# finegrain-ai/refiners

Measured on AMD Instinct MI355X. Metric: sdxl_base_1024px_images_per_sec_50_ddim_steps, higher is better.
Workload: dtype bf16; 1 GPU; SDXL-base UNet CFG step, 1024x1024 (latent 2x4x128x128, 77 text tokens), DDIM-50 + 2 LoRA r16 (722 Linears) + IP-Adapter; images_per_gpu=1, parallelism=replica x1 (independent prompts, weights broadcast once), hip_graph=True, lora_mode=fused, full=False

## Files before the change

### include/mi355x_refiners.h

```cpp
#ifndef MI355X_REFINERS_H
#define MI355X_REFINERS_H

#include <stdint.h>

#ifdef __cplusplus
extern "C" {
#endif

#define MI355X_ABI_VERSION 7

enum { MI355X_F32 = 0, MI355X_BF16 = 1 };

enum {
    MI355X_OK = 0,
    MI355X_EDTYPE = -1,
    MI355X_ESHAPE = -2,
    MI355X_ELAUNCH = -3,
    MI355X_EARG = -4
};

int mi355x_abi_version(void);
int mi355x_device_info(char* buf, int32_t buflen);

#define MI355X_MAX_SEG 3
// ... 10 lines not shown
    int32_t ups;
    int32_t H, W;
    int32_t asym;
    int32_t kblocked;
} mi355x_gemm_seg;

typedef struct {
    int32_t dtype;
    int32_t M, N;
    int32_t nseg;
    int32_t conv;
    int32_t B, OH, OW;
    mi355x_gemm_seg seg[MI355X_MAX_SEG];
    void* out;
    int64_t ldo;
    const void* bias;
    const void* rowbias;
    int64_t ld_rowbias;
    int32_t rows_per_group;
    int32_t geglu;
    const void* res;
    int64_t ldres;
    const void* zeros;
    int32_t tile;
    int32_t ksplit;
    void* ws;
    int64_t ws_bytes;
    const void* prefetch[MI355X_MAX_PREFETCH];
    int64_t prefetch_bytes[MI355X_MAX_PREFETCH];
    int32_t prefetch_blocks;
    int32_t out_kblocked;
    int32_t stages;
    int32_t nt_begin;
    void* out_t;
    int64_t ldt;
    const void* ln_stats;
    int32_t ln_parts;
    float ln_eps;
    const void* ln_s;
    const void* ln_c;
    void* stats_out;
    int32_t out_f32;
    const void* lora_a[3];
    int32_t lora_nb[3];
    int32_t lora_groups;
    int32_t lora_r;
    const void* lora_b;
    const void* lora_ls;
    const void* lora_lc;
    void* lora_t;
    int32_t* lora_flags;
    const int32_t* lora_epoch;
    float* colstats_out;
    void* sk_ws;
    int32_t* sk_flags;
    int32_t sk_slots;
} mi355x_gemm_args;

int mi355x_gemm(const mi355x_gemm_args* args, void* stream);
int mi355x_epoch_bump(int32_t* epoch, void* stream);

typedef struct {
    const void* k;
    int64_t ldk;
    int64_t k_batch_stride;
    const void* vt;
    int64_t ldvt;
    int64_t vt_batch_stride;
    int32_t Lk;
    float out_scale;
} mi355x_kv_stream;

typedef struct {
    int32_t dtype;
    int32_t B, H, D, Lq;
    int32_t nstream;
    const void* q;
    int64_t ldq;
    int64_t q_batch_stride;
    void* out;
    int64_t ldo;
    int64_t o_batch_stride;
    float scale;
    mi355x_kv_stream kv[2];
} mi355x_attn_args;

int mi355x_attention(const mi355x_attn_args* args, void* stream);

typedef struct {
    int32_t dtype;
    int32_t B, H, Lq, Lk;
    int32_t Dqk, Dv;
    int32_t causal;
    const void* q;
    int64_t ldq;
    int64_t q_batch_stride;
    const void* k;
    int64_t ldk;
    int64_t k_batch_stride;
    const void* vt;
    int64_t ldvt;
    int64_t vt_batch_stride;
    void* out;
    int64_t ldo;
    int64_t o_batch_stride;
    float scale;
    float out_scale;
} mi355x_attn_general_args;

int mi355x_attention_general(const mi355x_attn_general_args* args, void* stream);

typedef struct {
    int32_t dtype;
    int32_t M, C;
    const void* x;
    int64_t ldx;
    const void* gamma;
    const void* beta;
    float eps;
    void* out;
    int64_t ldo;
} mi355x_layernorm_args;

int mi355x_layernorm(const mi355x_layernorm_args* args, void* stream);

typedef struct {
    int32_t dtype;
    int32_t B, HW, C, G;
    const void* x;
    int64_t ldx;
    const void* gamma;
    const void* beta;
    float eps;
    int32_t silu;
    void* out;
    int64_t ldo;
    float* ws;
    const float* colstats;
    const void* x2;
    int64_t ldx2;
    int32_t C1;
    const float* colstats2;
} mi355x_groupnorm_args;

int64_t mi355x_groupnorm_ws_floats(int32_t B, int32_t HW, int32_t C);
int mi355x_groupnorm(const mi355x_groupnorm_args* args, void* stream);

int mi355x_nchw_to_nhwc(int32_t dtype, const void* x, void* out, int32_t B, int32_t C, int32_t HW, int64_t ldo, void* stream);
int mi355x_nhwc_to_nchw(int32_t dtype, const void* x, void* out, int32_t B, int32_t C, int32_t HW, int64_t ldx, void* stream);
int mi355x_im2col3x3_nchw(int32_t dtype, const void* x, void* out, int32_t B, int32_t C, int32_t H, int32_t W, int64_t ldo, void* stream);
int mi355x_patchify_nchw(int32_t dtype, const void* x, void* out, int32_t B, int32_t C, int32_t H, int32_t W, int32_t P, int64_t ldo, void* stream);
int mi355x_gather_rows(int32_t dtype, const void* x, int64_t ldx, const int32_t* idx, void* out, int64_t ldo, int64_t n_rows, int32_t C, void* stream);
int mi355x_relpos_pack(int32_t dtype, const void* src, int64_t lds, void* out, int64_t ldo, int64_t M, int32_t H, int32_t d, int32_t S1, int32_t S2,
                       int32_t Lp, int32_t Dq, void* stream);
int mi355x_pointwise_nchw(int32_t dtype, const void* x, const void* w, const void* bias, void* out, int32_t B, int32_t Ci, int32_t Co,
                          int64_t HW, void* stream);
int mi355x_concat2(int32_t dtype, const void* a, int64_t lda, int32_t C1, const void* b, int64_t ldb, int32_t C2,
                   void* out, int64_t ldo, int64_t M, void* stream);
int mi355x_axpby(int32_t dtype, const void* a, float alpha, const void* b, float beta, void* out, int64_t n, void* stream);
int mi355x_softmax_rows(int32_t dtype, const float* s, int64_t lds, void* out, int64_t ldo, int64_t M, int32_t L, int32_t Lp, float scale,
                        void* stream);
int mi355x_colsum_rows(int32_t dtype, const void* p, int64_t ldp, int32_t M, int32_t L, float* acc, int32_t accumulate, float scale, void* stream);
int mi355x_sag_degrade(int32_t dtype, const void* x, const void* eps, const float* mass, int32_t ah, int32_t aw, const float* coef, const float* w1,
                       int32_t ksize, void* out, int32_t n, int32_t C, int32_t h, int32_t w, void* stream);
int mi355x_silu(int32_t dtype, const void* x, void* out, int64_t n, void* stream);

// ... 56 lines not shown
```

### refiners_amd/csrc/attention.hip

```cpp
#include "common.cuh"
#include "../../include/mi355x_refiners.h"
#include <type_traits>

namespace {

struct KvP {
    const char* k;
    const char* vt;
    int64_t ldkb, kbsb;
    int64_t ldvtb, vtbsb;
    int Lk;
    float out_scale;
};

struct AttnP {
    int B, H, Lq, nstream;
    const char* q;
    int64_t ldqb, qbsb;
    char* out;
    int64_t ldob, obsb;
    float c;
    float thr;
    KvP kv[2];
    int qtiles;
    int xcd;
};

MI_DEV void xswap16(float& a, float& b) { asm("s_nop 1\n\tv_permlane16_swap_b32 %0, %1" : "+v"(a), "+v"(b)); }
MI_DEV void xswap32(float& a, float& b) { asm("s_nop 1\n\tv_permlane32_swap_b32 %0, %1" : "+v"(a), "+v"(b)); }
template <bool PL> MI_DEV float group_max(float x) {
    if constexpr (PL) {
        float a = x, b = x;
        xswap16(a, b);
        a = fmaxf(a, b), b = a;
        xswap32(a, b);
        return fmaxf(a, b);
    } else {
        x = fmaxf(x, __shfl_xor(x, 16));
        return fmaxf(x, __shfl_xor(x, 32));
    }
}
template <bool PL> MI_DEV float group_sum(float x) {
    if constexpr (PL) {
        float a = x, b = x;
        xswap16(a, b);
        a = a + b, b = a;
        xswap32(a, b);
        return a + b;
    } else {
        x += __shfl_xor(x, 16);
        return x + __shfl_xor(x, 32);
    }
}

template <typename T, int NW, int NSTREAM, bool GLDS, int NJQ, int RD = 2, int OPT = 0, int ABL = 0, int KVS = 1>
__global__ __launch_bounds__(NW * 64) __attribute__((amdgpu_waves_per_eu(sizeof(T) == 2 ? 2 : 1))) void attn_kernel(const AttnP p) {
    constexpr int D = 64, BKV = 64, BQW = 16 * NJQ;
    constexpr int ES = sizeof(T);
    constexpr int ROWB = D * ES;
    constexpr int CPR = ROWB / 16;
    constexpr int NTHR = NW * 64;
    constexpr int TILEB = 64 * ROWB;
    constexpr int STAGE = 2 * TILEB;
    constexpr int NST = GLDS ? 3 : 2;
    constexpr int PD = NST - 1;
    constexpr int LI = 64 * CPR / NTHR;
    constexpr int LPS = 2 * LI;
    constexpr int NS = D / DT<T>::KSTEP;
    constexpr bool IS_BF16 = (ES == 2);
    static_assert(64 * CPR % NTHR == 0, "loader mismatch");
    static_assert(KVS == 1 || (KVS == 2 && NSTREAM == 1 && !GLDS && NW % 2 == 0), "key-split: one stream, register-staged loader");
    constexpr int QW = NW / KVS;
    constexpr int TT = 4 / KVS;
    extern __shared__ __attribute__((aligned(16))) char smem[];

    const int tid = threadIdx.x, lane = tid & 63, wid = wave_id();
    const int g = lane >> 4, c16 = lane & 15;
    int bid = p.xcd ? xcd_remap(blockIdx.x, gridDim.x) : blockIdx.x;
    const int qt = bid % p.qtiles;
    bid /= p.qtiles;
    const int h = bid % p.H;
    const int b = bid / p.H;
    const int qg = KVS == 1 ? wid : wid % QW, kg = KVS == 1 ? 0 : wid / QW;
    const int q0 = qt * (BQW * QW) + qg * BQW;

    frag_t qf[NJQ][NS];
#pragma unroll
    for (int jq = 0; jq < NJQ; ++jq) {
        int qr = q0 + 16 * jq + c16;
        qr = qr < p.Lq ? qr : p.Lq - 1;
        const char* qp = p.q + (int64_t)b * p.qbsb + (int64_t)qr * p.ldqb + (int64_t)h * ROWB;
#pragma unroll
        for (int s = 0; s < NS; ++s) {
            if constexpr (ABL & 32) qf[jq][s] = frag_t{lane, s, jq, 0x3c003c00};
            else qf[jq][s] = *reinterpret_cast<const frag_t*>(qp + (4 * s + g) * 16);
        }
    }

    int lrow[LI], lcoff[LI], vrowd[LI];
#pragma unroll
    for (int it = 0; it < LI; ++it) {
        const int q = it * NTHR + tid, row = q / CPR, pch = q % CPR;
        lrow[it] = IS_BF16 ? k_row_key(row) : row;
        lcoff[it] = (pch ^ swz<ROWB>(row)) << 4;
        const int j = row >> 4, a = (row >> 2) & 3, bb = row & 3;
        vrowd[it] = 16 * a + 4 * j + bb;
    }
    frag_t kr[RD][LI], vr[RD][LI];
// ... 304 lines not shown
            }
        }

        if constexpr (KVS == 2) {
            constexpr int NV = 18 * NJQ;
            float* mg = reinterpret_cast<float*>(smem) + (qg * NV) * 64 + lane;
            if (kg == 1) {
#pragma unroll
                for (int jq = 0; jq < NJQ; ++jq) {
#pragma unroll
                    for (int i = 0; i < 4; ++i)
#pragma unroll
                        for (int r = 0; r < 4; ++r) mg[(jq * 18 + 4 * i + r) * 64] = o[i][jq][r];
                    mg[(jq * 18 + 16) * 64] = mrun[jq];
                    mg[(jq * 18 + 17) * 64] = lsum[jq];
                }
            }
            __syncthreads();
            if (kg == 0) {
#pragma unroll
                for (int jq = 0; jq < NJQ; ++jq) {
                    const float m1 = mg[(jq * 18 + 16) * 64], l1 = mg[(jq * 18 + 17) * 64];
                    const float m = fmaxf(mrun[jq], m1);
                    const float a0 = fast_exp2((mrun[jq] - m) * p.c), a1 = fast_exp2((m1 - m) * p.c);
                    lsum[jq] = lsum[jq] * a0 + l1 * a1;
#pragma unroll
                    for (int i = 0; i < 4; ++i)
#pragma unroll
                        for (int r = 0; r < 4; ++r) o[i][jq][r] = o[i][jq][r] * a0 + mg[(jq * 18 + 4 * i + r) * 64] * a1;
                }
            }
        }

#pragma unroll
        for (int jq = 0; jq < NJQ; ++jq) {
            float l;
            if constexpr (ONES) l = lacc[jq][0];
            else l = group_sum<(OPT & 1) != 0>(lsum[jq]);
            const float inv = kv.out_scale / l;
#pragma unroll
            for (int i = 0; i < 4; ++i) {
                if constexpr (NSTREAM > 1) res[i][jq] += o[i][jq] * inv;
                else res[i][jq] = o[i][jq] * inv;
            }
        }
    }

    constexpr int EPC = DT<T>::EPC;
#pragma unroll
    for (int jq = 0; jq < NJQ; ++jq) {
        const int qr = q0 + 16 * jq + c16;
        if (qr >= p.Lq || kg != 0) continue;
        if constexpr (ABL & 16) {
            if (res[0][jq][0] != 12345.678f) continue;
        }
        T* op = reinterpret_cast<T*>(p.out + (int64_t)b * p.obsb + (int64_t)qr * p.ldob + (int64_t)h * ROWB) + 16 * g;
        float v[16];
#pragma unroll
        for (int i = 0; i < 4; ++i)
#pragma unroll
            for (int r = 0; r < 4; ++r) v[4 * i + r] = res[i][jq][r];
#pragma unroll
        for (int c = 0; c < 16 / EPC; ++c) {
            Vec16<T> ov;
#pragma unroll
            for (int e = 0; e < EPC; ++e) ov.set(e, v[c * EPC + e]);
            store16<T>(op + c * EPC, ov);
        }
    }
}

typedef __amdgpu_buffer_rsrc_t rsrc_t;
MI_DEV rsrc_t make_rsrc(const char* base, int64_t bytes) {
    const uint64_t b = reinterpret_cast<uint64_t>(base);
    const uint32_t lo = __builtin_amdgcn_readfirstlane((uint32_t)b), hi = __builtin_amdgcn_readfirstlane((uint32_t)(b >> 32));
    const int64_t nb = bytes < 0x7ffffff0 ? bytes : 0x7ffffff0;
    const int n = __builtin_amdgcn_readfirstlane((int)nb);
    return __builtin_amdgcn_make_buffer_rsrc(reinterpret_cast<void*>(((uint64_t)hi << 32) | lo), (short)0, n, 0x00020000);
}
MI_DEV void blds16(rsrc_t rs, char* lds_wave_base, uint32_t voff, uint32_t soff) {
    __builtin_amdgcn_raw_ptr_buffer_load_lds(rs, (lptr_t)lds_wave_base, 16, (int)voff, (int)soff, 0, 0);
}

template <int NJQ, int SCHED, int ABL = 0, bool DMA = false, bool FOLD = false>
__global__ __launch_bounds__(256) __attribute__((amdgpu_waves_per_eu(2))) void attn_pipe_kernel(const AttnP p) {
    using T = bf16_t;
    constexpr int NW = 4, D = 64, BKV = 64, BQW = 16 * NJQ, ES = 2, ROWB = D * ES, CPR = ROWB / 16, NTHR = NW * 64, TILEB = 64 * ROWB;
    constexpr int LI = 64 * CPR / NTHR, NS = 2;
    extern __shared__ __attribute__((aligned(16))) char smem[];

    const int tid = threadIdx.x, lane = tid & 63, wid = wave_id();
    const int g = lane >> 4, c16 = lane & 15;
    int bid = p.xcd ? xcd_remap(blockIdx.x, gridDim.x) : blockIdx.x;
    const int qt = bid % p.qtiles;
    bid /= p.qtiles;
    const int h = bid % p.H;
    const int b = bid / p.H;
    const int q0 = qt * (BQW * NW) + wid * BQW;

    frag_t qf[NJQ][NS];
#pragma unroll
    for (int jq = 0; jq < NJQ; ++jq) {
        int qr = q0 + 16 * jq + c16;
        qr = qr < p.Lq ? qr : p.Lq - 1;
        const char* qp = p.q + (int64_t)b * p.qbsb + (int64_t)qr * p.ldqb + (int64_t)h * ROWB;
#pragma unroll
        for (int s = 0; s < NS; ++s) {
            qf[jq][s] = *reinterpret_cast<const frag_t*>(qp + (4 * s + g) * 16);
            if constexpr (FOLD) {
                bf16x8 qv = __builtin_bit_cast(bf16x8, qf[jq][s]);
#pragma unroll
                for (int e = 0; e < 8; ++e) qv[e] = (bf16_t)((float)qv[e] * p.c);
                qf[jq][s] = __builtin_bit_cast(frag_t, qv);
            }
        }
    }

    const KvP& kv = p.kv[0];
    const int Lk = kv.Lk;
    const int ntile = (Lk + BKV - 1) / BKV;
    const char* kbase = kv.k + (int64_t)b * kv.kbsb + (int64_t)h * ROWB;
    const char* vbase = kv.vt + (int64_t)h * D * kv.ldvtb + (int64_t)b * kv.vtbsb;
    char* const kbuf = smem;
    char* const vbuf = smem + 2 * TILEB;
    uint32_t koff[LI], koff_last[LI], voff[LI];
#pragma unroll
    for (int it = 0; it < LI; ++it) {
        const int q = it * NTHR + tid, row = q / CPR, pch = q % CPR;
        const int key = k_row_key(row);
        const int coff = (pch ^ swz<ROWB>(row)) << 4;
        const int last = Lk - 1 - (ntile - 1) * BKV;
        koff[it] = (uint32_t)(key * (int)kv.ldkb + coff);
        koff_last[it] = (uint32_t)((key < last ? key : last) * (int)kv.ldkb + coff);
        const int j = row >> 4, a = (row >> 2) & 3, bb = row & 3;
        voff[it] = (uint32_t)((16 * a + 4 * j + bb) * (int)kv.ldvtb + coff);
    }

    const rsrc_t krs = make_rsrc(kbase, (int64_t)(Lk - 1) * kv.ldkb + ROWB);
    const rsrc_t vrs = make_rsrc(vbase, (int64_t)(D - 1) * kv.ldvtb + (int64_t)ntile * BKV * ES);
    auto dma_k = [&](int tile, int buf) {
        const uint32_t soff = (uint32_t)(tile * BKV) * (uint32_t)kv.ldkb;
        const bool lastt = tile == ntile - 1;
#pragma unroll
        for (int it = 0; it < LI; ++it) blds16(krs, kbuf + buf * TILEB + (it * NTHR + wid * 64) * 16, lastt ? koff_last[it] : koff[it], soff);
    };
    auto dma_v = [&](int tile, int buf) {
        const uint32_t soff = (uint32_t)(tile * BKV * ES);
#pragma unroll
        for (int it = 0; it < LI; ++it) blds16(vrs, vbuf + buf * TILEB + (it * NTHR + wid * 64) * 16, voff[it], soff);
    };
    frag_t kr[LI], vr[LI];
    auto load_k = [&](int tile) {
        const char* base = kbase + (int64_t)tile * BKV * kv.ldkb;
        const bool lastt = tile == ntile - 1;
#pragma unroll
        for (int it = 0; it < LI; ++it) kr[it] = *reinterpret_cast<const frag_t*>(base + (lastt ? koff_last[it] : koff[it]));
    };
    auto load_v = [&](int tile) {
        const char* base = vbase + (int64_t)tile * BKV * ES;
#pragma unroll
        for (int it = 0; it < LI; ++it) vr[it] = *reinterpret_cast<const frag_t*>(base + voff[it]);
    };
    auto commit_k = [&](int buf) {
#pragma unroll
        for (int it = 0; it < LI; ++it) *reinterpret_cast<frag_t*>(kbuf + buf * TILEB + (it * NTHR + tid) * 16) = kr[it];
    };
    auto commit_v = [&](int buf) {
#pragma unroll
        for (int it = 0; it < LI; ++it) *reinterpret_cast<frag_t*>(vbuf + buf * TILEB + (it * NTHR + tid) * 16) = vr[it];
    };

    f32x4 o[4][NJQ], lacc[NJQ];
#pragma unroll
    for (int jq = 0; jq < NJQ; ++jq) {
        lacc[jq] = f32x4{0.f, 0.f, 0.f, 0.f};
#pragma unroll
        for (int i = 0; i < 4; ++i) o[i][jq] = f32x4{0.f, 0.f, 0.f, 0.f};
    }
    float mrun[NJQ];
#pragma unroll
    for (int jq = 0; jq < NJQ; ++jq) mrun[jq] = FOLD ? 0.f : -INFINITY;
    const frag_t ones = frag_t{0x3f803f80, 0x3f803f80, 0x3f803f80, 0x3f803f80};

    auto qk = [&](const char* ks, f32x4(&sn)[4][NJQ]) {
        frag_t kf[4][NS];
#pragma unroll
        for (int t = 0; t < 4; ++t)
#pragma unroll
            for (int s = 0; s < NS; ++s) kf[t][s] = lds_read_frag(ks, tile_off<ROWB>(16 * t + c16, 4 * s + g));
#pragma unroll
        for (int t = 0; t < 4; ++t) {
#pragma unroll
// ... 602 lines not shown
            const int kv0 = (sidx ? sl - nt0 : sl) * BKV;
            if (Lk - kv0 <= 32) tile(smem + sl * STAGE, kv0, Lk, std::true_type{});
            else tile(smem + sl * STAGE, kv0, Lk, std::false_type{});
        }
    }
    finish(p.kv[NSTREAM - 1].out_scale);

#pragma unroll
    for (int jq = 0; jq < NJQ; ++jq) {
        const int qr = q0 + 16 * jq + c16;
        if (qr >= p.Lq) continue;
        T* op = reinterpret_cast<T*>(p.out + (int64_t)b * p.obsb + (int64_t)qr * p.ldob + (int64_t)h * ROWB) + 16 * g;
#pragma unroll
        for (int c = 0; c < 2; ++c) {
            Vec16<T> ov;
#pragma unroll
            for (int e = 0; e < 8; ++e) ov.set(e, res[(c * 8 + e) >> 2][jq][e & 3]);
            store16<T>(op + c * 8, ov);
        }
    }
}

int g_attn_short_q16 = 0;

int g_attn_short_dma = 1;

template <typename T, int NSTREAM, int NJQ, bool DMA>
auto short_kernel_of() {
    if constexpr (DMA) return attn_short_dma_kernel<NSTREAM, NJQ>;
    else return attn_short_kernel<T, NSTREAM, NJQ>;
}

template <typename T, int NSTREAM, int NJQ = 2, bool DMA = false>
int launch_attn_short(const AttnP& p0, int xcd, hipStream_t stream) {
    if constexpr (sizeof(T) == 2 && !DMA) {
        bool ok = g_attn_short_dma != 0;
        for (int s = 0; s < p0.nstream; ++s) ok = ok && 64 * p0.kv[s].ldkb < 0x7fffffff && 64 * p0.kv[s].ldvtb < 0x7fffffff;
        if (ok) return launch_attn_short<T, NSTREAM, NJQ, true>(p0, xcd, stream);
    }
    constexpr int LDS = 3 * 2 * 64 * 64 * sizeof(T);
    auto kfn = short_kernel_of<T, NSTREAM, NJQ, DMA>();
    static bool attr_set = false;
    if (!attr_set) {
        (void)hipFuncSetAttribute(reinterpret_cast<const void*>(kfn), hipFuncAttributeMaxDynamicSharedMemorySize, LDS);
        attr_set = true;
    }
    AttnP p = p0;
    constexpr int BQ = 64 * NJQ;
    p.qtiles = (p.Lq + BQ - 1) / BQ;
    p.xcd = xcd;
    hipLaunchKernelGGL(kfn, dim3(p.qtiles * p.H * p.B), dim3(256), LDS, stream, p);
    return hipGetLastError() == hipSuccess ? MI355X_OK : MI355X_ELAUNCH;
}

int g_attn_glds = 0;
int g_attn_depth = 1;
int g_attn_xcd = 1;
int g_attn_opt = 13;
int g_attn_abl = 0;
int g_attn_kvs = 0;

template <typename T, int NW, int NSTREAM, bool GLDS, int NJQ = 2, int RD = 2, int OPT = 0, int ABL = 0, int KVS = 1>
int launch_attn(const AttnP& p0, hipStream_t stream) {
    constexpr int LDS = (GLDS ? 3 : 2) * 2 * 64 * 64 * sizeof(T);
    auto kfn = attn_kernel<T, NW, NSTREAM, GLDS, NJQ, RD, OPT, ABL, KVS>;
    static bool attr_set = false;
    if (!attr_set) {
        (void)hipFuncSetAttribute(reinterpret_cast<const void*>(kfn), hipFuncAttributeMaxDynamicSharedMemorySize, LDS);
        attr_set = true;
    }
    AttnP p = p0;
    constexpr int BQ = 16 * NJQ * NW / KVS;
    p.qtiles = (p.Lq + BQ - 1) / BQ;
    p.xcd = g_attn_xcd;
    const int grid = p.qtiles * p.H * p.B;
    hipLaunchKernelGGL(kfn, dim3(grid), dim3(NW * 64), LDS, stream, p);
    return hipGetLastError() == hipSuccess ? MI355X_OK : MI355X_ELAUNCH;
}

int g_attn_pipe = 3;

int g_attn_pipe_fold = 0;

template <int NJQ, int SCHED, int ABL = 0, bool DMA = false, bool FOLD = false>
int launch_attn_pipe(const AttnP& p0, hipStream_t stream) {
    constexpr int LDS = 4 * 64 * 64 * 2;
    auto kfn = attn_pipe_kernel<NJQ, SCHED, ABL, DMA, FOLD>;
    static bool attr_set = false;
    if (!attr_set) {
        (void)hipFuncSetAttribute(reinterpret_cast<const void*>(kfn), hipFuncAttributeMaxDynamicSharedMemorySize, LDS);
        attr_set = true;
    }
    AttnP p = p0;
    constexpr int BQ = 16 * NJQ * 4;
    p.qtiles = (p.Lq + BQ - 1) / BQ;
    p.xcd = g_attn_xcd;
    hipLaunchKernelGGL(kfn, dim3(p.qtiles * p.H * p.B), dim3(256), LDS, stream, p);
    return hipGetLastError() == hipSuccess ? MI355X_OK : MI355X_ELAUNCH;
}

int g_attn_nw = 0;

template <typename T, int NW, int OPT>
int launch_attn_opt(const AttnP& p, hipStream_t stream) {
    if constexpr (NW != 2) {
        if (g_attn_depth == 2) {
            if constexpr (OPT != 2) {
                if (p.nstream == 2) return launch_attn<T, NW, 2, false, 2, 2, OPT>(p, stream);
            }
            if (p.nstream == 1) return launch_attn<T, NW, 1, false, 2, 2, OPT>(p, stream);
        }
    }
    if (p.nstream == 2) return launch_attn<T, NW, 2, false, 2, 1, OPT>(p, stream);
    return launch_attn<T, NW, 1, false, 2, 1, OPT>(p, stream);
}

template <typename T, int NW>
int launch_attn_nw(const AttnP& p, hipStream_t stream) {
    if constexpr (NW == 4 && sizeof(T) == 2) {
#ifdef MI355X_ATTN_PIPE_ABL
        if (g_attn_pipe && p.nstream == 1 && g_attn_abl != 0) {
            switch (g_attn_abl) {
                case 1: return launch_attn_pipe<2, 1, 1>(p, stream);
                case 2: return launch_attn_pipe<2, 1, 2>(p, stream);
                case 4: return launch_attn_pipe<2, 1, 4>(p, stream);
                case 6: return launch_attn_pipe<2, 1, 6>(p, stream);
                case 8: return launch_attn_pipe<2, 1, 8>(p, stream);
                case 16: return launch_attn_pipe<2, 1, 16>(p, stream);
                case 24: return launch_attn_pipe<2, 1, 24>(p, stream);
                case 32: return launch_attn_pipe<2, 1, 32>(p, stream);
                case 33: return launch_attn_pipe<2, 1, 33>(p, stream);
                case 39: return launch_attn_pipe<2, 1, 39>(p, stream);
                case 63: return launch_attn_pipe<2, 1, 63>(p, stream);
                case 128: return launch_attn_pipe<2, 1, 0, true>(p, stream);
                case 129: return launch_attn_pipe<2, 1, 1, true>(p, stream);
                case 134: return launch_attn_pipe<2, 1, 6, true>(p, stream);
                case 144: return launch_attn_pipe<2, 1, 16, true>(p, stream);
                case 167: return launch_attn_pipe<2, 1, 39, true>(p, stream);
                case 136: return launch_attn_pipe<2, 1, 8, true>(p, stream);
                case 152: return launch_attn_pipe<2, 1, 24, true>(p, stream);
                case 175: return launch_attn_pipe<2, 1, 47, true>(p, stream);
                case 191: return launch_attn_pipe<2, 1, 63, true>(p, stream);
                default: return MI355X_EARG;
            }
        }
#endif
    }
    if (g_attn_glds) {
        if (p.nstream == 2) return launch_attn<T, NW, 2, true>(p, stream);
        return launch_attn<T, NW, 1, true>(p, stream);
    }
    if constexpr (NW == 4 && sizeof(T) == 2) {
        if (g_attn_abl && p.nstream == 1) {
            switch (g_attn_abl) {
                case 1: return launch_attn<T, 4, 1, false, 2, 1, 0, 1>(p, stream);
                case 2: return launch_attn<T, 4, 1, false, 2, 1, 0, 2>(p, stream);
                case 4: return launch_attn<T, 4, 1, false, 2, 1, 0, 4>(p, stream);
                case 8: return launch_attn<T, 4, 1, false, 2, 1, 0, 8>(p, stream);
                case 6: return launch_attn<T, 4, 1, false, 2, 1, 0, 6>(p, stream);
                case 14: return launch_attn<T, 4, 1, false, 2, 1, 0, 14>(p, stream);
                case 15: return launch_attn<T, 4, 1, false, 2, 1, 0, 15>(p, stream);
                case 31: return launch_attn<T, 4, 1, false, 2, 1, 0, 31>(p, stream);
                case 63: return launch_attn<T, 4, 1, false, 2, 1, 0, 63>(p, stream);
                case 127: return launch_attn<T, 4, 1, false, 2, 1, 0, 127>(p, stream);
                case 16: return launch_attn<T, 4, 1, false, 2, 1, 0, 16>(p, stream);
                default: return MI355X_EARG;
            }
        }
    }
    if constexpr (NW == 4 && sizeof(T) == 2) {
        if (g_attn_pipe && p.nstream == 1 && g_attn_abl == 0 && g_attn_kvs != 2) {
            const int64_t wg128 = (int64_t)((p.Lq + 127) / 128) * p.H * p.B;
            const bool q16 = g_attn_kvs == 3 || (g_attn_kvs == 0 && wg128 <= 640 && p.kv[0].Lk >= 256);
            if (g_attn_pipe == 2) return q16 ? launch_attn_pipe<1, 0>(p, stream) : launch_attn_pipe<2, 0>(p, stream);
            if (g_attn_pipe == 3) {
                const bool dma_ok = (int64_t)p.kv[0].Lk * p.kv[0].ldkb < 0x7fffffff && 64 * p.kv[0].ldvtb < 0x7fffffff;
                if (dma_ok && g_attn_pipe_fold) return q16 ? launch_attn_pipe<1, 1, 0, true, true>(p, stream) : launch_attn_pipe<2, 1, 0, true, true>(p, stream);
                if (dma_ok) return q16 ? launch_attn_pipe<1, 1, 0, true>(p, stream) : launch_attn_pipe<2, 1, 0, true>(p, stream);
            }
            return q16 ? launch_attn_pipe<1, 1>(p, stream) : launch_attn_pipe<2, 1>(p, stream);
        }
    }
    if constexpr (NW == 4) {
        const int64_t wg128 = (int64_t)((p.Lq + 127) / 128) * p.H * p.B;
        const bool short_grid = wg128 <= 384 && p.kv[0].Lk >= 256;
        if (p.nstream == 1 && (g_attn_kvs == 3 || (g_attn_kvs == 0 && short_grid))) {
            if constexpr (sizeof(T) == 2) {
                switch (g_attn_opt) {
                    case 5: return launch_attn<T, 4, 1, false, 1, 1, 5>(p, stream);
                    case 9: return launch_attn<T, 4, 1, false, 1, 1, 9>(p, stream);
                    case 13: return launch_attn<T, 4, 1, false, 1, 1, 13>(p, stream);
                    default: break;
                }
            }
            return launch_attn<T, 4, 1, false, 1, 1, 1>(p, stream);
        }
        if (p.nstream == 1 && g_attn_kvs == 2) return (g_attn_opt & 1) ? launch_attn<T, 4, 1, false, 2, 1, 1, 0, 2>(p, stream) : launch_attn<T, 4, 1, false, 2, 1, 0, 0, 2>(p, stream);
    }
    if constexpr (NW == 4 && sizeof(T) == 2) {
        if (p.nstream == 1) {
            switch (g_attn_opt) {
                case 5: return launch_attn<T, 4, 1, false, 2, 1, 5>(p, stream);
                case 9: return launch_attn<T, 4, 1, false, 2, 1, 9>(p, stream);
                case 13: return launch_attn<T, 4, 1, false, 2, 1, 13>(p, stream);
                default: break;
            }
        }
    }
    switch (g_attn_opt & 3) {
        case 1: return launch_attn_opt<T, NW, 1>(p, stream);
        case 2: return launch_attn_opt<T, NW, 2>(p, stream);
        case 3: return launch_attn_opt<T, NW, 3>(p, stream);
        default: return launch_attn_opt<T, NW, 0>(p, stream);
    }
}

int g_attn_short = 1;

template <typename T>
int launch_attn_t(const AttnP& p, hipStream_t stream) {
    if (g_attn_short && !g_attn_glds && g_attn_nw == 0 && g_attn_abl == 0 && g_attn_kvs != 2) {
        int tiles = 0;
        for (int s = 0; s < p.nstream; ++s) tiles += (p.kv[s].Lk + 63) / 64;
        if (tiles <= 3) {
            const int64_t wg128 = (int64_t)((p.Lq + 127) / 128) * p.H * p.B;
            if (g_attn_short_q16 == 2 || (g_attn_short_q16 == 0 && wg128 <= 640))
                return p.nstream == 2 ? launch_attn_short<T, 2, 1>(p, g_attn_xcd, stream) : launch_attn_short<T, 1, 1>(p, g_attn_xcd, stream);
            return p.nstream == 2 ? launch_attn_short<T, 2>(p, g_attn_xcd, stream) : launch_attn_short<T, 1>(p, g_attn_xcd, stream);
        }
    }
    int nw = g_attn_nw;
    if (nw == 0) nw = 4;
    if (nw == 14) return p.nstream == 2 ? launch_attn<T, 4, 2, false, 1, 1>(p, stream) : launch_attn<T, 4, 1, false, 1, 1>(p, stream);
    if (nw == 18) return p.nstream == 2 ? launch_attn<T, 8, 2, false, 1, 1>(p, stream) : launch_attn<T, 8, 1, false, 1, 1>(p, stream);
    return nw == 2 ? launch_attn_nw<T, 2>(p, stream) : launch_attn_nw<T, 4>(p, stream);
}

inline bool al16(const void* p) { return (reinterpret_cast<uintptr_t>(p) & 15) == 0; }

}

extern "C" int mi355x_attention_set_nw(int v) {
    g_attn_nw = v;
    return MI355X_OK;
}

extern "C" int mi355x_attention_set_glds(int v) {
    g_attn_glds = v;
    return MI355X_OK;
}

extern "C" int mi355x_attention_set_pipeline(int tiles_in_flight, int xcd_aware) {
    const int d = tiles_in_flight & 15;
    if (d == 1 || d == 2) g_attn_depth = d;
    g_attn_opt = (tiles_in_flight >> 4) & 15;
    g_attn_abl = (tiles_in_flight >> 8) & 255;
    g_attn_kvs = (tiles_in_flight >> 16) & 3;
    g_attn_short = ((tiles_in_flight >> 18) & 1) ? 0 : 1;
    g_attn_pipe = (tiles_in_flight >> 19) & 3;
    g_attn_pipe_fold = (tiles_in_flight >> 21) & 1;
    g_attn_short_q16 = (tiles_in_flight >> 23) & 3;
    g_attn_short_dma = ((tiles_in_flight >> 25) & 1) ? 0 : 1;
    if (xcd_aware >= 0) g_attn_xcd = xcd_aware ? 1 : 0;
    return MI355X_OK;
}

extern "C" int mi355x_attention(const mi355x_attn_args* a, void* stream) {
    if (!a || !a->q || !a->out) return MI355X_EARG;
    if (a->dtype != MI355X_F32 && a->dtype != MI355X_BF16) return MI355X_EDTYPE;
    if (a->D != 64 || a->B <= 0 || a->H <= 0 || a->Lq <= 0 || a->nstream < 1 || a->nstream > 2) return MI355X_ESHAPE;
    const int es = a->dtype == MI355X_F32 ? 4 : 2;
    if (!al16(a->q) || !al16(a->out) || (a->ldq * es) % 16 || (a->ldo * es) % 16 || (a->q_batch_stride * es) % 16 ||
        (a->o_batch_stride * es) % 16)
        return MI355X_ESHAPE;
    AttnP p{};
    p.B = a->B;
    p.H = a->H;
    p.Lq = a->Lq;
    p.nstream = a->nstream;
    p.q = static_cast<const char*>(a->q);
    p.ldqb = a->ldq * es;
    p.qbsb = a->q_batch_stride * es;
    p.out = static_cast<char*>(a->out);
    p.ldob = a->ldo * es;
    p.obsb = a->o_batch_stride * es;
    p.c = a->scale * 1.44269504088896340736f;
    p.thr = p.c > 0.f ? 8.0f / p.c : 0.f;
    for (int s = 0; s < a->nstream; ++s) {
        const mi355x_kv_stream& k = a->kv[s];
        if (!k.k || !k.vt || k.Lk <= 0) return MI355X_ESHAPE;
        if (!al16(k.k) || !al16(k.vt) || (k.ldk * es) % 16 || (k.ldvt * es) % 16 || (k.k_batch_stride * es) % 16 ||
            (k.vt_batch_stride * es) % 16)
            return MI355X_ESHAPE;
        p.kv[s].k = static_cast<const char*>(k.k);
        p.kv[s].vt = static_cast<const char*>(k.vt);
        p.kv[s].ldkb = k.ldk * es;
        p.kv[s].kbsb = k.k_batch_stride * es;
        p.kv[s].ldvtb = k.ldvt * es;
        p.kv[s].vtbsb = k.vt_batch_stride * es;
        p.kv[s].Lk = k.Lk;
        p.kv[s].out_scale = k.out_scale;
    }
    hipStream_t st = static_cast<hipStream_t>(stream);
    if (a->dtype == MI355X_F32) return launch_attn_t<float>(p, st);
    return launch_attn_t<bf16_t>(p, st);
}
```

### refiners_amd/csrc/gemm.hip

```cpp
#include <climits>

#include "gemm8_kernel.cuh"
#include "gemm_kernel.cuh"

namespace mi355x {

int g_pf_blocks = 64;
int g_pf_mode = 1;
int g_tile = 0;
int g_stages = 0;
int g_lora_dbg = 0;
int g_sk_g = 0;
int g_g8_persist = 1;

namespace {
inline bool aligned16(const void* p) { return (reinterpret_cast<uintptr_t>(p) & 15) == 0; }
}

}

using namespace mi355x;

extern "C" int mi355x_set_option(const char* name, int value);
extern "C" int mi355x_set_option(const char* name, int value) {
    if (!name) return MI355X_EARG;
    if (name[0] == 'g' && name[1] == 'n') {
        extern int g_gn_wgs, g_gn_unroll;
        if (name[2] == 'w') g_gn_wgs = value;
        else g_gn_unroll = value;
        return MI355X_OK;
    }
    if (name[0] == 'g' && name[1] == '8') {
        g_g8_persist = value;
        return MI355X_OK;
    }
    if (name[0] == 's' && name[1] == 'k') {
        g_sk_g = value;
        return MI355X_OK;
    }
    if (name[0] == 's') {
        g_stages = value;
        return MI355X_OK;
    }
    if (name[0] == 'p') {
        if (name[2] == 'b') g_pf_blocks = value < 0 ? 0 : (value + 7) / 8 * 8;
        else g_pf_mode = value;
        return MI355X_OK;
    }
    if (name[0] == 'l') {
        g_lora_dbg = value;
        return MI355X_OK;
    }
    if (name[0] == 't') {
        g_tile = value;
        return MI355X_OK;
    }
    return MI355X_EARG;
}

static int g_stat_g8 = 0, g_stat_g8_lora = 0, g_stat_g9 = 0, g_stat_g11 = 0, g_stat_g12 = 0;
extern "C" int mi355x_get_stat(const char* name);
extern "C" int mi355x_get_stat(const char* name) {
    if (!name) return MI355X_EARG;
    if (name[0] == 'g' && name[1] == '8') return name[2] == 'l' ? g_stat_g8_lora : g_stat_g8;
    if (name[0] == 'g' && name[1] == '9') return g_stat_g9;
    if (name[0] == 'g' && name[1] == '1' && name[2] == '1') return g_stat_g11;
    if (name[0] == 'g' && name[1] == '1' && name[2] == '2') return g_stat_g12;
    return MI355X_EARG;
}

namespace {
__global__ void epoch_bump_kernel(int* e) {
    const int v = *e + 1;
    *e = v == 0 ? 1 : v;
}
}

extern "C" int mi355x_epoch_bump(int32_t* epoch, void* stream) {
    if (!epoch) return MI355X_EARG;
    hipLaunchKernelGGL(epoch_bump_kernel, dim3(1), dim3(1), 0, static_cast<hipStream_t>(stream), epoch);
    return hipGetLastError() == hipSuccess ? MI355X_OK : MI355X_ELAUNCH;
}

extern "C" int mi355x_gemm(const mi355x_gemm_args* a, void* stream) {
    if (!a) return MI355X_EARG;
    const bool has_t = a->out_t != nullptr;
    if (!a->out && !(has_t && a->nt_begin == 0)) return MI355X_EARG;
    if (a->dtype != MI355X_F32 && a->dtype != MI355X_BF16) return MI355X_EDTYPE;
    if (a->M <= 0 || a->N <= 0 || a->nseg < 1 || a->nseg > MI355X_MAX_SEG) return MI355X_ESHAPE;
    const int es = a->dtype == MI355X_F32 ? 4 : 2;
    const int bke = 128 / es;
    GemmP p{};
    p.M = a->M;
    p.N = a->N;
    p.nseg = a->nseg;
    p.OH = a->OH;
    p.OW = a->OW;
    if (a->conv) {
        if (!a->zeros || a->B <= 0 || a->OH <= 0 || a->OW <= 0 || (int64_t)a->B * a->OH * a->OW != a->M) return MI355X_ESHAPE;
    }
    for (int s = 0; s < a->nseg; ++s) {
        const mi355x_gemm_seg& g = a->seg[s];
        if (!g.x || !g.w || g.k <= 0 || g.k % bke) return MI355X_ESHAPE;
        const bool wkb = g.kblocked & 1, xkb = (g.kblocked & 2) != 0;
        if (xkb && a->conv) return MI355X_ESHAPE;
        if (!aligned16(g.x) || !aligned16(g.w) || (!xkb && (g.ldx * es) % 16) || (!wkb && (g.ldw * es) % 16)) return MI355X_ESHAPE;
        SegP& d = p.seg[s];
        d.wkb = wkb ? 1 : 0;
        d.xkb = xkb ? 1 : 0;
        d.x = static_cast<const char*>(g.x);
        d.w = static_cast<const char*>(g.w);
        d.ldxb = g.ldx * es;
        d.ldwb = g.ldw * es;
        {
            const int64_t taps = a->conv ? (int64_t)g.ksize * g.ksize : 1, kbytes = (int64_t)g.k * es, nkb_all = taps * (g.k / bke);
            const int64_t xrows = a->conv ? (int64_t)a->B * g.H * g.W : (int64_t)a->M;
            d.xbytes = xkb ? nkb_all * a->M * 128 : (xrows - 1) * d.ldxb + kbytes;
            d.wbytes = wkb ? nkb_all * a->N * 128 : ((int64_t)a->N - 1) * d.ldwb + taps * kbytes;
        }
        if (a->conv) {
            if ((g.ksize != 1 && g.ksize != 3) || (g.stride != 1 && g.stride != 2) || (g.ups != 1 && g.ups != 2)) return MI355X_ESHAPE;
            if (g.H <= 0 || g.W <= 0) return MI355X_ESHAPE;
            d.cpb = g.k / bke;
            d.nkb = g.ksize * g.ksize * d.cpb;
            d.ksize = g.ksize;
            d.pad = g.asym ? 0 : g.ksize / 2;
            d.stride = g.stride;
            d.ups_shift = g.ups == 2 ? 1 : 0;
            d.H = g.H;
            d.W = g.W;
        } else {
            d.cpb = 1;
            d.nkb = g.k / bke;
            d.ksize = 1;
            d.pad = 0;
            d.stride = 1;
            d.ups_shift = 0;
        }
    }
    p.out = static_cast<char*>(a->out);
    p.ldo = a->ldo;
    p.bias = static_cast<const char*>(a->bias);
    p.rowbias = static_cast<const char*>(a->rowbias);
    p.ld_rowbias = a->ld_rowbias;
    p.rows_per_group = a->rows_per_group > 0 ? a->rows_per_group : 1;
    p.geglu = a->geglu == 1 ? 1 : 0;
// ... 130 lines not shown
```

### refiners_amd/csrc/gemm_epilogue.cuh

```cuda
#pragma once
#include "gemm_params.cuh"

enum : unsigned { EPI_LN = 1, EPI_RB = 2, EPI_GELU = 4, EPI_GEGLU = 8, EPI_RES = 16, EPI_F32 = 32, EPI_ST = 64, EPI_CS = 128, EPI_ALL = 255 };
#define EPIF(bit, x) (((F) & (bit)) != 0 && (x))

namespace mi355x {

template <int BM, int NTHR_ALL>
MI_DEV void ln_rowstat(const GemmP& p, int m0, int tid_all, float* rowstat) {
    constexpr int TPR = NTHR_ALL / BM;
    static_assert(TPR >= 1 && (TPR & (TPR - 1)) == 0 && TPR <= 8, "threads per row");
    const int row = tid_all / TPR, sub = tid_all % TPR;
    const int m = min(m0 + row, p.M - 1);
    float cn = 0.f, mean = 0.f, m2 = 0.f;
    constexpr int MAXP = 24;
    const float* sp = p.ln_stats + (int64_t)m * 2;
    const int64_t pstride = (int64_t)p.M * 2;
    f32x2 st[MAXP];
#pragma unroll
    for (int i = 0; i < MAXP; ++i) {
        const int part = sub + i * TPR;
        st[i] = part < p.ln_parts ? *reinterpret_cast<const f32x2*>(sp + part * pstride) : f32x2{0.f, 0.f};
    }
#pragma unroll
// ... 325 lines not shown
    const T* bias = reinterpret_cast<const T*>(p.bias);
    const T* rowbias = reinterpret_cast<const T*>(p.rowbias);
    const T* res = reinterpret_cast<const T*>(p.res);
    float s1[4] = {0.f, 0.f, 0.f, 0.f}, s2[4] = {0.f, 0.f, 0.f, 0.f};
    const bool full4 = n + 4 <= p.N;
    if (n < p.N) {
        f32x4 part[2][MAXS];
#pragma unroll
        for (int r = 0; r < 2; ++r) {
            const int m = min(bm * 32 + ty * 2 + r, p.M - 1);
#pragma unroll
            for (int s = 0; s < MAXS; ++s) {
                part[r][s] = f32x4{0.f, 0.f, 0.f, 0.f};
                if (s < p.ksplit) {
                    const float* pp = p.partial + ((int64_t)s * p.M + m) * p.N + n;
                    if (full4) part[r][s] = *reinterpret_cast<const f32x4*>(pp);
                    else
                        for (int q = 0; q < 4; ++q)
                            if (n + q < p.N) part[r][s][q] = pp[q];
                }
            }
        }
#pragma unroll
        for (int r = 0; r < 2; ++r) {
            const int m = bm * 32 + ty * 2 + r;
            if (m >= p.M) break;
            float v[4] = {0.f, 0.f, 0.f, 0.f};
#pragma unroll
            for (int s = 0; s < MAXS; ++s)
                if (s < p.ksplit) v[0] += part[r][s][0], v[1] += part[r][s][1], v[2] += part[r][s][2], v[3] += part[r][s][3];
            for (int s = MAXS; s < p.ksplit; ++s) {
                const float* pp = p.partial + ((int64_t)s * p.M + m) * p.N + n;
                for (int q = 0; q < 4; ++q)
                    if (n + q < p.N) v[q] += pp[q];
            }
#pragma unroll
            for (int q = 0; q < 4; ++q) {
                const int nn = n + q;
                if (nn >= p.N) break;
                float val = v[q];
                if (bias) val += to_f32(bias[nn]);
                if (rowbias) val += to_f32(rowbias[(int64_t)(m / p.rows_per_group) * p.ld_rowbias + nn]);
                if (p.gelu) val = epi_act(p.gelu, val);
                if (res) val += to_f32(res[(int64_t)m * p.ldres + nn]);
                const T o = from_f32<T>(val);
                out[(int64_t)m * p.ldo + nn] = o;
                const float f = to_f32(o);
                s1[q] += f;
                s2[q] += f * f;
            }
        }
    }
    if (p.colstats) {
        if (ty > 0) {
#pragma unroll
            for (int q = 0; q < 4; ++q) {
                red[ty - 1][tx][q] = s1[q];
                red[ty - 1][tx][4 + q] = s2[q];
            }
        }
        __syncthreads();
        if (ty == 0 && n < p.N) {
#pragma unroll
            for (int q = 0; q < 4; ++q) {
                if (n + q >= p.N) break;
                float a = s1[q], b = s2[q];
#pragma unroll
                for (int j = 0; j < 15; ++j) {
                    a += red[j][tx][q];
                    b += red[j][tx][4 + q];
                }
                f32x2 st = {a, b};
                *reinterpret_cast<f32x2*>(p.colstats + ((int64_t)bm * p.N + n + q) * 2) = st;
            }
        }
    }
}

extern int g_pf_blocks;
extern int g_pf_mode;
extern int g_tile;
extern int g_stages;
extern int g_lora_dbg;


inline void plan_grid(GemmP& q, int BM, int BN, bool conv, int kg) {
    const GemmP& p = q;
    q.tiles_n = (p.N + BN - 1) / BN;
    q.tiles_m = (p.M + BM - 1) / BM;
    double kx = 0, kw = 0;
    for (int sgi = 0; sgi < p.nseg; ++sgi) {
        const SegP& sg = p.seg[sgi];
        kw += sg.nkb;
        kx += conv ? (double)sg.nkb / (sg.ksize * sg.ksize) : (double)sg.nkb;
    }
    const double bx_ = (double)p.M * kx, bw_ = (double)p.N * kw;
    double best = bx_ + 8.0 * bw_;
    q.pn = 0;
    q.hm = q.hn = 0;
    if (8.0 * bx_ + bw_ < best) {
        best = 8.0 * bx_ + bw_;
        q.pn = -1;
    }
    for (int pm = 2; pm <= 4; pm *= 2) {
        const int pn = 8 / pm;
        if (q.tiles_m % pm || q.tiles_n % pn) continue;
        const double cost = pn * bx_ + pm * bw_;
        if (cost < best) {
            best = cost;
            q.pn = pn;
            q.hm = q.tiles_m / pm;
            q.hn = q.tiles_n / pn;
        }
    }
    q.grid0 = q.tiles_m * q.tiles_n;
    bool any_pf = false;
    for (int i = 0; i < MI355X_MAX_PREFETCH; ++i) any_pf = any_pf || (q.pf_ptr[i] && q.pf_bytes[i] > 0);
    if (!any_pf || g_pf_blocks == 0) q.pf_blocks = 0;
    else if (q.pf_blocks <= 0) q.pf_blocks = g_pf_blocks;
    q.pf_blocks = (q.pf_blocks + 7) / 8 * 8;
    if (kg > 1) q.pf_blocks = (q.pf_blocks / 2 + 7) / 8 * 8;
    q.pf_mode = g_pf_mode;
}

}
```

### refiners_amd/csrc/gemm_kernel.cuh

```cuda
#pragma once
#include "gemm_epilogue.cuh"
#include "gemm_lora_producer.cuh"

namespace mi355x {

#ifndef MI355X_GEMM_PRIO
#define MI355X_GEMM_PRIO 1
#endif
#ifndef MI355X_LORA_TT
#define MI355X_LORA_TT 1
#endif
#ifndef MI355X_LORA_TT_HOOKS
#define MI355X_LORA_TT_HOOKS 0
#endif
#ifndef MI355X_LORA64_WAVES
#define MI355X_LORA64_WAVES 4
#endif
template <typename T, int BM, int BN, bool LORA> constexpr int gemm_min_waves() {
    if (!LORA || sizeof(T) != 2) return 1;
    return BM * BN == 128 * 128 ? 2 : BM * BN == 64 * 64 ? MI355X_LORA64_WAVES : BM == 128 ? 3 : 2;
}

template <typename T, int BM, int BN, int WM, int WN, bool CONV, int NSTAGE, int KG = 1, bool LORA = false>
__global__ __launch_bounds__(WM* WN * 64 * KG) __attribute__((amdgpu_waves_per_eu(gemm_min_waves<T, BM, BN, LORA>()))) void gemm_kernel(const GemmP p) {
    constexpr int NW = WM * WN;
    constexpr int NTHR = NW * 64;
    constexpr int NTHR_ALL = NTHR * KG;
    constexpr int MT = BM / WM / 16, NT = BN / WN / 16;
    constexpr int XI = BM * 8 / NTHR, WI = BN * 8 / NTHR;
    constexpr int XBYTES = BM * 128, WBYTES = BN * 128, STAGE = XBYTES + WBYTES;
    static_assert(NSTAGE >= 2 && NSTAGE <= 4, "2..4 LDS stages");
    static_assert(!LORA || (KG == 1 && NTHR == 256 && WN == 2 && NSTAGE == 2), "in-launch LoRA: 4 waves as 2 x 2, two LDS stages");
    static_assert(KG == 1 || KG == 2, "one or two K groups");
    constexpr int WNE = 16 * NT;
    constexpr int WME = 16 * MT;
    static_assert(BM * 8 % NTHR == 0 && BN * 8 % NTHR == 0, "tile/thread mismatch");
    extern __shared__ __attribute__((aligned(16))) char smem[];
    float* rowstat = reinterpret_cast<float*>(smem + KG * NSTAGE * STAGE);
    char* const lora_b0 = smem + KG * NSTAGE * STAGE + (p.ln_stats ? BM * 8 : 0);

    const int tid_all = threadIdx.x, wid_all = wave_id();
    const int kg = KG > 1 ? wid_all / NW : 0;
    const int tid = tid_all - kg * NTHR, lane = tid & 63, wid = wid_all - kg * NW;
    const int g = lane >> 4, c16 = lane & 15;
    const int wm = wid / WN, wn = wid % WN;
    char* const smem_g = smem + kg * (NSTAGE * STAGE);
    if ((int)blockIdx.x < p.pf_blocks) {
        int acc = 0;
        const int64_t stride = (int64_t)p.pf_blocks * NTHR_ALL * 64;
        constexpr int U = 8;
#pragma unroll
        for (int sp = 0; sp < MI355X_MAX_PREFETCH; ++sp) {
            const char* base = p.pf_ptr[sp];
            const int64_t bytes = base ? p.pf_bytes[sp] : 0;
            for (int64_t off = ((int64_t)blockIdx.x * NTHR_ALL + tid_all) * 64; off < bytes; off += stride * U) {
                int v[U];
#pragma unroll
                for (int u = 0; u < U; ++u) {
                    const int64_t o = off + u * stride;
                    const int* src = reinterpret_cast<const int*>(base + (o < bytes ? o : off));
                    v[u] = p.pf_mode == 2 ? __builtin_nontemporal_load(src) : *src;
                }
#pragma unroll
                for (int u = 0; u < U; ++u) acc ^= v[u];
            }
        }
        if (acc == 0x5a5a1234 && p.pf_bytes[0] < 0) *reinterpret_cast<int*>(p.out) = acc;
        return;
    }
    int bid = (int)blockIdx.x - p.pf_blocks;
    bool ttile = false;
    int tt_tag = 0;
    if constexpr (LORA && !CONV) {
        if (p.lora_tt && bid < p.lp_blocks) {
            if ((p.lora_dbg & 1) || bid >= p.tiles_m) return;
            ttile = true;
            tt_tag = *p.lora_epoch;
        }
    }
    if constexpr (LORA) {
        if (!ttile && bid < p.lp_blocks) {
            if ((p.lora_dbg & 1) || bid >= (p.M + LORA_PM - 1) / LORA_PM * p.lora_groups) return;
            constexpr int RING = KG * NSTAGE * (BM + BN) * 128;
            constexpr int PB1 = (LORA_PM + 32) * 128, PB2 = (LORA_PM + 64) * 128, PB4 = (LORA_PM + 128) * 128;
            constexpr int P1 = RING / PB1 < 8 ? RING / PB1 : 8, P2 = RING / PB2 < 8 ? RING / PB2 : 8, P4 = RING / PB4;
            if (p.lora_r == 32) lora_producer<T, CONV, 1, P1>(p, bid);
            else if (p.lora_r == 64) lora_producer<T, CONV, 2, P2>(p, bid);
            else if constexpr (P4 >= 2) lora_producer<T, CONV, 4, (P4 < 8 ? P4 : 8)>(p, bid);
            return;
        }
        if (!ttile) bid -= p.lp_blocks;
    }
    const int split = p.ksplit > 1 ? bid / p.grid0 : 0;
    const int bx = bid - split * p.grid0;
    int tm, tn;
    if (ttile) {
        tm = bid;
        tn = 0;
    } else if (p.pn > 0) {
        const int xcd = bx & 7, idx = bx >> 3;
        const int rm = xcd / p.pn, rn = xcd - rm * p.pn;
        const int lm = idx / p.hn, ln = idx - lm * p.hn;
        tm = rm * p.hm + lm;
        tn = rn * p.hn + ln;
    } else {
        const int id = xcd_remap(bx, p.grid0);
        if (p.pn == 0) {
            tm = id / p.tiles_n;
            tn = id - tm * p.tiles_n;
        } else {
            tn = id / p.tiles_m;
            tm = id - tn * p.tiles_m;
        }
    }
    if (tm >= p.tiles_m || tn >= p.tiles_n) return;
    const int m0 = tm * BM, n0 = tn * BN;
    const bool tr = !CONV && !ttile && n0 >= p.nt_begin;

    int xm[XI];
    int xcoff[XI];
    int xb[XI], xoy[XI], xox[XI];
    bool xvalid[XI];
#pragma unroll
    for (int it = 0; it < XI; ++it) {
        const int q = it * NTHR + tid, row = q >> 3, pch = q & 7;
        xcoff[it] = (pch ^ swz<128>(row)) << 4;
        int mr = row;
        if (!CONV && tr) {
            const int rl = row % WME;
            mr = (row - rl) + 4 * MT * ((rl >> 2) & 3) + 4 * (rl >> 4) + (rl & 3);
        }
        const int m = m0 + mr;
        xvalid[it] = m < p.M;
        xm[it] = m < p.M ? m : p.M - 1;
        if constexpr (CONV) {
            const int ohw = p.OH * p.OW;
            const int b = xm[it] / ohw, rem = xm[it] - b * ohw;
            xb[it] = b;
            xoy[it] = rem / p.OW;
            xox[it] = rem - xoy[it] * p.OW;
        }
    }
    int wnrow[WI], wcoff[WI];
#pragma unroll
    for (int it = 0; it < WI; ++it) {
        const int q = it * NTHR + tid, row = q >> 3, pch = q & 7;
        wcoff[it] = (pch ^ swz<128>(row)) << 4;
        const int rl = row % WNE, j = rl >> 4, a = (rl >> 2) & 3, b = rl & 3;
        const int n = n0 + (tr ? row : (row - rl) + 4 * NT * a + 4 * j + b);
        wnrow[it] = n < p.N ? n : p.N - 1;
        if (LORA && ttile) wnrow[it] = n < p.lora_groups * p.lora_r ? n : 0;
    }

    f32x4 acc[MT][NT];
#pragma unroll
    for (int i = 0; i < MT; ++i)
#pragma unroll
        for (int j = 0; j < NT; ++j) acc[i][j] = f32x4{0.f, 0.f, 0.f, 0.f};
    const int lgi = LORA && !ttile ? (p.lora_groups > 1 && n0 >= p.lora_nb[1] ? 1 : 0) + (p.lora_groups > 2 && n0 >= p.lora_nb[2] ? 1 : 0) : 0;
    const bool lora_tail = LORA && !ttile && split == 0 && !(p.lora_dbg & 4);

    int seg = 0, kb = 0;
    int total_kb = 0;
    for (int s = 0; s < p.nseg; ++s) total_kb += p.seg[s].nkb;
    if (p.ksplit > 1) {
        const int first = split * p.kb_per_split;
// ... 322 lines not shown
        for (int i = 0; i < MT; ++i)
#pragma unroll
            for (int j = 0; j < NT; ++j) {
                const f32x4 o = ex[(i * NT + j) * 64];
                acc[i][j][0] += o[0], acc[i][j][1] += o[1], acc[i][j][2] += o[2], acc[i][j][3] += o[3];
            }
    } else if (p.ln_stats) {
        __syncthreads();
    }

    if constexpr (LORA && !CONV) {
        if (ttile) {
            constexpr int RUN = 4 * NT;
            const int nv = wn * WNE + RUN * g;
            const int rsh = p.lora_r == 32 ? 5 : p.lora_r == 64 ? 6 : 7;
            const int gi = nv >> rsh, r0 = nv & (p.lora_r - 1);
            const float* lsl = reinterpret_cast<const float*>(lora_b0);
            if (gi < p.lora_groups) {
                char* tg = p.lora_t + gi * p.lora_gs;
#pragma unroll
                for (int i = 0; i < MT; ++i) {
                    const int mrow = wm * WME + 16 * i + c16, m = m0 + mrow;
                    if (m >= p.M) continue;
                    float v[RUN];
#pragma unroll
                    for (int j = 0; j < NT; ++j)
#pragma unroll
                        for (int r = 0; r < 4; ++r) v[4 * j + r] = acc[i][j][r];
                    if (p.ln_stats) {
                        const float mean = rowstat[2 * mrow], inv = 1.0f / rowstat[2 * mrow + 1];
#pragma unroll
                        for (int c = 0; c < RUN / 4; ++c) {
                            const f32x4 sa = *reinterpret_cast<const f32x4*>(lsl + gi * p.lora_r + r0 + 4 * c);
                            const f32x4 ca = *reinterpret_cast<const f32x4*>(lsl + 256 + gi * p.lora_r + r0 + 4 * c);
#pragma unroll
                            for (int e = 0; e < 4; ++e) v[4 * c + e] = (v[4 * c + e] - mean * sa[e]) + ca[e] * inv;
                        }
                    }
                    char* dst = tg + ((int64_t)m * p.lora_r + r0) * (int)sizeof(T);
                    if constexpr (sizeof(T) == 4) {
#pragma unroll
                        for (int c = 0; c < RUN / 2; ++c) st_agent8(dst + 8 * c, __builtin_bit_cast(uint64_t, f32x2{v[2 * c], v[2 * c + 1]}));
                    } else {
#pragma unroll
                        for (int c = 0; c < RUN / 4; ++c) {
                            const bf16x4 b4 = {(bf16_t)v[4 * c], (bf16_t)v[4 * c + 1], (bf16_t)v[4 * c + 2], (bf16_t)v[4 * c + 3]};
                            st_agent8(dst + 8 * c, __builtin_bit_cast(uint64_t, b4));
                        }
                    }
                }
            }
            asm volatile("s_waitcnt vmcnt(0)" ::: "memory");
            __syncthreads();
            constexpr int FB = BM / LORA_PM;
            if (tid < p.lora_groups * FB) {
                const int nfl = (p.M + LORA_PM - 1) / LORA_PM, fg = tid / FB, fb = m0 / LORA_PM + tid % FB;
                if (fb < nfl) __hip_atomic_store(p.lora_flags + fg * nfl + fb, tt_tag, __ATOMIC_RELAXED, __HIP_MEMORY_SCOPE_AGENT);
            }
            return;
        }
    }

    tile_epilogue<T, MT, NT, BM, CONV>(p, acc, rowstat, m0, n0, wm, wn, lane, tr, split);
}

template <typename T, int BM, int BN, int WM, int WN, bool CONV, int NSTAGE, int KG = 1, bool LORA = false>
int launch_cfg(const GemmP& p, hipStream_t stream) {
    constexpr int LDS0 = KG * NSTAGE * (BM + BN) * 128 + BM * 8 + (LORA ? BN * LORA_RC * (int)sizeof(T) : 0);
    constexpr int LDS = LDS0;
    static_assert(LDS <= 160 * 1024, "LDS budget");
    static_assert(KG == 1 || (BM / WM / 16) * (BN / WN / 16) * WM * WN * 1024 <= KG * NSTAGE * (BM + BN) * 128, "partial-tile exchange must fit the stage buffers");
    auto kfn = gemm_kernel<T, BM, BN, WM, WN, CONV, NSTAGE, KG, LORA>;
    static bool attr_set[64] = {};
    int dev = 0;
    (void)hipGetDevice(&dev);
    if (dev >= 0 && dev < 64 && !attr_set[dev]) {
        (void)hipFuncSetAttribute(reinterpret_cast<const void*>(kfn), hipFuncAttributeMaxDynamicSharedMemorySize, LDS);
        attr_set[dev] = true;
    }
    GemmP q = p;
    plan_grid(q, BM, BN, CONV, KG);
    q.lora_dbg = g_lora_dbg;
    q.lora_tt = 0;
    if constexpr (LORA && !CONV && KG == 1) {
        const int mode = (g_lora_dbg & 64) ? 0 : (g_lora_dbg & 128) ? 2 : MI355X_LORA_TT;
        if (q.lora_groups * q.lora_r <= BN && q.ksplit <= 1 && q.nseg == 1 && (mode == 2 || (mode == 1 && q.lora_groups > 1))) q.lora_tt = 1;
    }
    q.lp_blocks = !LORA ? 0 : q.lora_tt ? (q.tiles_m + 7) / 8 * 8 : ((q.M + LORA_PM - 1) / LORA_PM * q.lora_groups + 7) / 8 * 8;
    const int grid = q.pf_blocks + q.lp_blocks + q.grid0 * (q.ksplit > 1 ? q.ksplit : 1);
    hipLaunchKernelGGL(kfn, dim3(grid), dim3(WM * WN * 64 * KG), q.ln_stats ? LDS : LDS - BM * 8, stream, q);
    if (q.ksplit > 1) {
        const int rb = ((q.M + 31) / 32) * ((q.N + 63) / 64);
        hipLaunchKernelGGL((splitk_reduce_kernel<T>), dim3(rb), dim3(256), 0, stream, q);
    }
    return hipGetLastError() == hipSuccess ? MI355X_OK : MI355X_ELAUNCH;
}

inline int pick_tile(const GemmP& p, bool conv) {
    if ((g_tile >= 1 && g_tile <= 4) || g_tile == 6) return g_tile;
    if ((p.tile_hint >= 1 && p.tile_hint <= 4) || p.tile_hint == 6) return p.tile_hint;
    const int64_t b128 = (int64_t)((p.M + 127) / 128) * ((p.N + 127) / 128);
    if (conv) return 3;
    if (p.geglu) return 1;
    if (b128 <= 256) return 4;
    if (b128 < 1000) return 2;
    return 1;
}
inline int pick_stages(const GemmP& p) {
    if (g_stages >= 2 && g_stages <= 4) return g_stages;
    if (p.stage_hint >= 2 && p.stage_hint <= 4) return p.stage_hint;
    return 2;
}

template <typename T, int BM, int BN, bool CONV>
int launch_stages(const GemmP& p, int stages, hipStream_t stream) {
    switch (stages) {
        case 2: return launch_cfg<T, BM, BN, 2, 2, CONV, 2>(p, stream);
        case 4: return launch_cfg<T, BM, BN, 2, 2, CONV, 4>(p, stream);
        default: return launch_cfg<T, BM, BN, 2, 2, CONV, 3>(p, stream);
    }
}

template <typename T, bool CONV>
int launch_tile(const GemmP& p, hipStream_t stream) {
    int tile = pick_tile(p, CONV);
    if (p.geglu && (tile == 2 || tile == 4)) tile = 3;
    if (p.colstats && tile == 6) tile = 1;
    const int st = pick_stages(p);
    if (p.lora_b) {
        if (p.lora_r > 64 && (tile == 2 || tile == 4)) tile = tile == 2 ? 1 : 3;
        if constexpr (CONV) {
            return tile == 1 ? launch_cfg<T, 128, 128, 2, 2, true, 2, 1, true>(p, stream) : launch_cfg<T, 64, 128, 2, 2, true, 2, 1, true>(p, stream);
        } else {
            switch (tile) {
                case 2: return launch_cfg<T, 128, 64, 2, 2, false, 2, 1, true>(p, stream);
                case 3: return launch_cfg<T, 64, 128, 2, 2, false, 2, 1, true>(p, stream);
                case 4: return launch_cfg<T, 64, 64, 2, 2, false, 2, 1, true>(p, stream);
                default: return launch_cfg<T, 128, 128, 2, 2, false, 2, 1, true>(p, stream);
            }
        }
    }
#ifdef MI355X_PROBE_T10
    if constexpr (!CONV) {
        if (g_tile == 10 || p.tile_hint == 10) return launch_cfg<T, 128, 96, 4, 1, false, 2>(p, stream);
        if (g_tile == 11 || p.tile_hint == 11) return launch_cfg<T, 128, 96, 4, 1, false, 3>(p, stream);
        if (g_tile == 12 || p.tile_hint == 12) return launch_cfg<T, 64, 64, 2, 1, false, 2>(p, stream);
        if (g_tile == 13 || p.tile_hint == 13) return launch_cfg<T, 64, 64, 2, 1, false, 3>(p, stream);
        if (g_tile == 14 || p.tile_hint == 14) return launch_cfg<T, 128, 64, 2, 1, false, 2>(p, stream);
        if (g_tile == 15 || p.tile_hint == 15) return launch_cfg<T, 128, 64, 2, 1, false, 3>(p, stream);
    }
#endif
    switch (tile) {
        case 1: return launch_stages<T, 128, 128, CONV>(p, st, stream);
        case 2: return launch_stages<T, 128, 64, CONV>(p, st, stream);
        case 3: return launch_stages<T, 64, 128, CONV>(p, st, stream);
        case 6: return launch_cfg<T, 128, 128, 2, 2, CONV, 2, 2>(p, stream);
        default: return launch_stages<T, 64, 64, CONV>(p, st, stream);
    }
}

int launch_conv_f32(const GemmP& p, hipStream_t stream);
int launch_conv_bf16(const GemmP& p, hipStream_t stream);

}
```

### refiners_amd/csrc/gemm_lora_producer.cuh

```cuda
#pragma once
#include "gemm_epilogue.cuh"

namespace mi355x {

constexpr int LORA_RC = 32;
constexpr int LORA_PM = 32;
constexpr int LORA_RMAX = 128;

template <typename T, bool CONV, int RI, int PST>
__device__ __forceinline__ void lora_producer(const GemmP& p, int q, int tid_in = -1, char* lds = nullptr) {
    extern __shared__ __attribute__((aligned(16))) char smem_all[];
    char* const smem = lds ? lds : smem_all;
    constexpr int NTHR = 256, PXB = LORA_PM * 128, PSTAGE = PXB + 32 * RI * 128, PD = PST - 1, PL = 1 + RI;
    static_assert(PST >= 2 && PST <= 8, "LoRA producer: 2..8 stages");
    const int tid = tid_in >= 0 ? tid_in : (int)threadIdx.x, lane = tid & 63, wid = __builtin_amdgcn_readfirstlane(tid >> 6), g = lane >> 4, c16 = lane & 15;
    const int npb = (p.M + LORA_PM - 1) / LORA_PM;
    const int pgi = q / npb, tm = q - pgi * npb, m0 = tm * LORA_PM;
    const int tag = *p.lora_epoch;
    if (p.lora_dbg & 32) __builtin_amdgcn_s_setprio(3);
    const SegP& sp = p.seg[0];
    const int nkb = sp.nkb;
    const int row = tid >> 3, pch = tid & 7;
    const int xcoff = (pch ^ swz<128>(row)) << 4;
    const bool xvalid = m0 + row < p.M;
    const int xm = xvalid ? m0 + row : p.M - 1;
    int xb = 0, xoy = 0, xox = 0;
    if constexpr (CONV) {
        const int ohw = p.OH * p.OW;
        xb = xm / ohw;
        const int rem = xm - xb * ohw;
        xoy = rem / p.OW;
        xox = rem - xoy * p.OW;
    }
    const char* xbase = nullptr;
    int64_t xoff = 0, woff = 0;
    const int64_t xstep = CONV ? 128 : (sp.xkb ? (int64_t)p.M * 128 : 128), wstep = (int64_t)p.lora_r * 128;
    int tap = 0, cb = 0;
    auto set_tap = [&]() __attribute__((always_inline)) {
        int dy = tap / sp.ksize, dx = tap - dy * sp.ksize;
        dy -= sp.pad;
        dx -= sp.pad;
        const int iy = xoy * sp.stride + dy, ix = xox * sp.stride + dx;
        const int HH = sp.H << sp.ups_shift, WW = sp.W << sp.ups_shift;
        const bool ok = xvalid && iy >= 0 && iy < HH && ix >= 0 && ix < WW;
        const int sy = iy >> sp.ups_shift, sx = ix >> sp.ups_shift;
        const int64_t pix = ((int64_t)xb * sp.H + sy) * sp.W + sx;
        xbase = ok ? sp.x + pix * sp.ldxb + xcoff : nullptr;
    };
    if constexpr (CONV) set_tap();
    else xbase = sp.x + (sp.xkb ? (int64_t)xm * 128 : (int64_t)xm * sp.ldxb) + xcoff;
    const char* pw[RI];
#pragma unroll
    for (int j = 0; j < RI; ++j) {
        const int qq = j * NTHR + tid, r = qq >> 3, c = qq & 7;
        pw[j] = p.lora_a[pgi] + (int64_t)r * 128 + ((c ^ swz<128>(r)) << 4);
    }
    int kb = 0;
    auto issue_p = [&](int buf) __attribute__((always_inline)) {
        char* st = smem + buf * PSTAGE;
        const char* src;
        if constexpr (CONV) src = xbase ? xbase + (int64_t)cb * 128 : p.zeros + xcoff;
        else src = xbase + xoff;
        glds16(src, st + wid * 64 * 16);
#pragma unroll
        for (int j = 0; j < RI; ++j) glds16(pw[j] + woff, st + PXB + (j * NTHR + wid * 64) * 16);
        ++kb;
        woff += wstep;
        if constexpr (CONV) {
            if (++cb == sp.cpb) {
                cb = 0;
                ++tap;
                if (kb < nkb) set_tap();
            }
        } else {
            xoff += xstep;
        }
    };
    const int rb = wid & 1, rg = wid >> 1;
    const int mrow = 16 * rb + c16, m = m0 + mrow;
    float mean = 0.f, inv = 1.f;
    constexpr int MAXP = 48;
    f32x2 lst[MAXP];
    const float* sp2 = p.ln_stats ? p.ln_stats + (int64_t)min(m, p.M - 1) * 2 : nullptr;
    const int64_t pstride = (int64_t)p.M * 2;
    if (sp2) {
#pragma unroll
        for (int i = 0; i < MAXP; ++i) lst[i] = i < p.ln_parts ? *reinterpret_cast<const f32x2*>(sp2 + i * pstride) : f32x2{0.f, 0.f};
    }
#pragma unroll
    for (int s0 = 0; s0 < PD; ++s0)
        if (s0 < nkb) issue_p(s0);
    if (sp2) {
        float m2 = 0.f, cn = 0.f;
#pragma unroll
        for (int i = 0; i < MAXP; ++i)
            if (i < p.ln_parts) stat_merge(cn, mean, m2, 32.f, lst[i][0], lst[i][1]);
        for (int part = MAXP; part < p.ln_parts; ++part) {
            const f32x2 s2 = *reinterpret_cast<const f32x2*>(sp2 + part * pstride);
            stat_merge(cn, mean, m2, 32.f, s2[0], s2[1]);
        }
        inv = sqrtf(m2 / cn + p.ln_eps);
    }
    f32x4 ta[RI];
#pragma unroll
    for (int j = 0; j < RI; ++j) ta[j] = f32x4{0.f, 0.f, 0.f, 0.f};
    for (int t = 0; t < nkb; ++t) {
        if (t + PD <= nkb) wait_vm<(PD - 1) * PL>();
        else wait_vm0();
        asm volatile("s_waitcnt lgkmcnt(0)" ::: "memory");
        __builtin_amdgcn_s_barrier();
        if (t + PD < nkb) issue_p((t + PD) % PST);
        const char* st = smem + (t % PST) * PSTAGE;
#pragma unroll
        for (int kk = 0; kk < 2; ++kk) {
            const frag_t xf = lds_read_frag(st, tile_off<128>(16 * rb + c16, 4 * kk + g));
#pragma unroll
            for (int j = 0; j < RI; ++j) {
                const frag_t af = lds_read_frag(st + PXB, tile_off<128>((rg * RI + j) * 16 + c16, 4 * kk + g));
                mma_step<T>(ta[j], af, xf);
            }
        }
    }
    char* tg = p.lora_t + pgi * p.lora_gs;
#pragma unroll
    for (int j = 0; j < RI; ++j) {
        const int r0 = (rg * RI + j) * 16 + 4 * g;
        f32x4 v = ta[j];
        if (p.ln_stats) {
            const f32x4 sa = *reinterpret_cast<const f32x4*>(p.lora_ls + pgi * p.lora_r + r0), ca = *reinterpret_cast<const f32x4*>(p.lora_lc + pgi * p.lora_r + r0);
#pragma unroll
            for (int e = 0; e < 4; ++e) v[e] = (v[e] - mean * sa[e]) + ca[e] * inv;
        }
        if (m < p.M) {
            char* dst = tg + ((int64_t)m * p.lora_r + r0) * (int)sizeof(T);
            if constexpr (sizeof(T) == 4) {
                st_agent8(dst, __builtin_bit_cast(uint64_t, f32x2{v[0], v[1]}));
                st_agent8(dst + 8, __builtin_bit_cast(uint64_t, f32x2{v[2], v[3]}));
            } else {
                const bf16x4 b4 = {(bf16_t)v[0], (bf16_t)v[1], (bf16_t)v[2], (bf16_t)v[3]};
                st_agent8(dst, __builtin_bit_cast(uint64_t, b4));
            }
        }
    }
    asm volatile("s_waitcnt vmcnt(0)" ::: "memory");
    __syncthreads();
    if (tid == 0) __hip_atomic_store(p.lora_flags + pgi * npb + tm, tag, __ATOMIC_RELAXED, __HIP_MEMORY_SCOPE_AGENT);
}

}
```

### refiners_amd/csrc/gemm_params.cuh

```cuda
#pragma once
#include <type_traits>

#include "../../include/mi355x_refiners.h"
#include "common.cuh"

namespace mi355x {

struct SegP {
    const char* x;
    const char* w;
    int64_t ldxb;
    int64_t ldwb;
    int nkb;
    int cpb;
    int ksize, stride, ups_shift, H, W;
    int wkb, xkb;
    int64_t xbytes, wbytes;
    int pad;
};

struct GemmP {
    int M, N, nseg;
    int OH, OW;
    SegP seg[MI355X_MAX_SEG];
    char* out;
    int64_t ldo;
    const char* bias;
    const char* rowbias;
    int64_t ld_rowbias;
    int rows_per_group;
    int geglu;
    int gelu;
    const char* res;
    int64_t ldres;
    const char* zeros;
    int tiles_m, tiles_n;
    int ksplit, kb_per_split, grid0;
    float* partial;
    int tile_hint;
    int stage_hint;
    int out_kb;
    int nt_begin;
    char* out_t;
    int64_t ldt;
    const float* ln_stats;
    int ln_parts;
    float ln_eps;
    const float* ln_s;
    const float* ln_c;
    float* stats_out;
    float* colstats;
    int out_f32;
    const char* lora_a[3];
    int lora_nb[3];
    int lora_groups;
    int lora_r;
    const char* lora_b;
    const float* lora_ls;
    const float* lora_lc;
    char* lora_t;
    int* lora_flags;
    const int* lora_epoch;
    int lp_blocks;
    int lora_tt;
    int64_t lora_gs;
    int lora_dbg;
    const char* pf_ptr[MI355X_MAX_PREFETCH];
    int64_t pf_bytes[MI355X_MAX_PREFETCH];
    int pf_blocks, pf_mode;
    int pn, hm, hn;
    int vec_ok;
    int sk_g, sk_nk, sk_order, sk_cap, sk_mode;
    int mix_nbig, mix_rb, mix_cb;
    float* sk_ws;
    int* sk_flags;
};

MI_DEV void stat_merge(float& n, float& mean, float& m2, float nb, float mb, float m2b) {
    const float nt = n + nb;
    if (nt > 0.f) {
        const float d = mb - mean, f = nb / nt;
        mean += d * f;
        m2 += m2b + d * d * n * f;
        n = nt;
    }
}

template <int CTRL> MI_DEV float dpp_f32(float v) {
    return __builtin_bit_cast(float, __builtin_amdgcn_update_dpp(0, __builtin_bit_cast(int, v), CTRL, 0xF, 0xF, true));
}
template <int RUN> MI_DEV void colsum16(float (&a)[RUN], float (&b)[RUN], int c16) {
    static_assert(RUN == 4 || RUN == 8 || RUN == 16, "4, 8 or 16 columns per lane");
    constexpr int ROW_MIRROR = 0x140, ROW_HALF_MIRROR = 0x141, QUAD_XOR2 = 0x4E, QUAD_XOR1 = 0xB1;
    auto step = [&](auto ctrl, int w) __attribute__((always_inline)) {
        constexpr int CTRL = decltype(ctrl)::value;
        const bool up = (c16 & w) != 0;
#pragma unroll
        for (int e = 0; e < RUN / 2; ++e) {
            if (e < w) {
                const float sa = up ? a[e] : a[e + w], sb = up ? b[e] : b[e + w];
                const float ka = up ? a[e + w] : a[e], kb = up ? b[e + w] : b[e];
                a[e] = ka + dpp_f32<CTRL>(sa);
                b[e] = kb + dpp_f32<CTRL>(sb);
            }
        }
    };
    if constexpr (RUN == 16) {
        step(std::integral_constant<int, ROW_MIRROR>{}, 8);
    } else {
#pragma unroll
        for (int e = 0; e < RUN; ++e) {
            a[e] += dpp_f32<ROW_MIRROR>(a[e]);
            b[e] += dpp_f32<ROW_MIRROR>(b[e]);
        }
    }
    if constexpr (RUN == 4) {
#pragma unroll
        for (int e = 0; e < 4; ++e) {
            a[e] += dpp_f32<ROW_HALF_MIRROR>(a[e]);
            b[e] += dpp_f32<ROW_HALF_MIRROR>(b[e]);
        }
    } else {
        step(std::integral_constant<int, ROW_HALF_MIRROR>{}, 4);
    }
    step(std::integral_constant<int, QUAD_XOR2>{}, 2);
    step(std::integral_constant<int, QUAD_XOR1>{}, 1);
}

MI_DEV void st_agent8(void* p, uint64_t v) { __hip_atomic_store(reinterpret_cast<uint64_t*>(p), v, __ATOMIC_RELAXED, __HIP_MEMORY_SCOPE_AGENT); }

}
```

### refiners_amd/engine/lowering.py

```python
from __future__ import annotations

import os

import math
from dataclasses import dataclass, field
from typing import Any, Callable, Optional

import torch
import torch.nn.functional as F
from torch import Tensor, nn

from .. import native

from .packing import Act, CatAct, ConvSpec, LinSpec, LoraPack, PackCache, Pool, Unsupported, _expect, cname, isa, kids, launches


class Lowering:
    def __init__(self, device: torch.device, dtype: torch.dtype, cache: Optional[PackCache] = None, lora_mode: str = "fused") -> None:
        assert lora_mode in ("fused", "merged")
        self.lora_mode = lora_mode
        self.kblock_policy = int(os.environ.get("REFINERS_AMD_KBLOCK", "2"))
        self.ln_fuse = os.environ.get("REFINERS_AMD_LN_FUSE", "1") != "0"
        self.qkv_merge = os.environ.get("REFINERS_AMD_QKV_MERGE", "1") != "0"
        self.lora_inlaunch = os.environ.get("REFINERS_AMD_LORA_INLAUNCH", "1") != "0"
        self.gn_stats = os.environ.get("REFINERS_AMD_GN_STATS", "1") != "0"
        self._cs_buf: list[Tensor] = []
        self._lsync: Any = None
        self._sk = native.StreamK(device)
        self._bumped: set[int] = set()
        self.device, self.dtype = device, dtype
        self.es = 4 if dtype == torch.float32 else 2
        self.kblk = 128 // self.es
        self.cache = cache or PackCache()
        self.cache.build_device = device
        self.step_pool = Pool(device, dtype)
        self.prologue_pool = Pool(device, dtype)
        self.pool = self.step_pool
        self.prologue: list = []
        self.step: list = []
        self._target = self.step
        self.stats = {"fallback_nodes": [], "lora_sites": 0, "ip_sites": 0}

    class _Section:
        def __init__(self, low: "Lowering", ops: list) -> None:
            self.low, self.ops = low, ops

        def __enter__(self) -> None:
            self.saved = (self.low._target, self.low.pool)
            self.low._target = self.ops
            self.low.pool = self.low.prologue_pool if self.ops is self.low.prologue else self.low.step_pool
            self.rec = native.recording(self.ops)
            self.rec.__enter__()
            self.sk_saved = native.set_streamk(self.low._sk)

        def __exit__(self, *exc: object) -> None:
            native.set_streamk(self.sk_saved)
            self.rec.__exit__(*exc)
            self.low._target, self.low.pool = self.saved

    def in_prologue(self) -> "Lowering._Section":
        return Lowering._Section(self, self.prologue)

    def in_step(self) -> "Lowering._Section":
        return Lowering._Section(self, self.step)

    def python(self, fn: Callable[[], None], what: str) -> None:
        self._target.append((None, fn, what, ()))

    def cvt(self, t: Tensor) -> Tensor:
        if t.device == self.device and t.dtype == self.dtype and t.is_contiguous() and t.data_ptr() % 16 == 0:
            return t.detach()
        return t.detach().to(device=self.device, dtype=self.dtype).contiguous()

    def _w(self, t: Optional[Tensor], tag: str = "cvt") -> Optional[Tensor]:
        if t is None:
            return None
        return self.cache.get((tag,) + PackCache.ident(t), lambda: self.cvt(t))

    def _unwrap_lora(self, node: Any, leaf_cls: str) -> tuple[Any, list[Any]]:
        if isa(node, "LoraAdapter"):
            ch = kids(node)
            _expect(len(ch) >= 1 and isa(ch[0], leaf_cls), f"LoraAdapter target is {cname(ch[0]) if ch else None}, wanted {leaf_cls}")
            loras = ch[1:]
            for lr in loras:
                c = kids(lr)
                _expect(isa(lr, "Lora") and len(c) == 3 and isa(c[2], "Multiply") and c[2].bias == 0.0, "unexpected Lora layout")
            return ch[0], loras
        _expect(isa(node, leaf_cls), f"expected {leaf_cls}-like node, got {cname(node)}")
        return node, []

    def _lora_pack_linear(self, loras: list[Any], n_out: int, k_in: int, row_perm: Optional[Tensor]) -> Optional[LoraPack]:
        if not loras:
            return None
        downs = [kids(lr)[0].weight for lr in loras]
        ups = [kids(lr)[1].weight for lr in loras]
        scales = tuple(float(kids(lr)[2].scale) for lr in loras)
        key = ("lora",) + PackCache.ident(*downs, *ups) + scales + (None if row_perm is None else "geglu",)

        def make() -> LoraPack:
            rt = sum(d.shape[0] for d in downs)
            rpad = (rt + self.kblk - 1) // self.kblk * self.kblk
            a = torch.zeros(rpad, k_in, device=self.device, dtype=self.dtype)
            bs = torch.zeros(n_out, rpad, device=self.device, dtype=self.dtype)
            o = 0
            for d, u, s in zip(downs, ups, scales):
                r = d.shape[0]
                _expect(tuple(d.shape) == (r, k_in) and tuple(u.shape) == (n_out, r), "LoRA shape does not match its target")
                a[o : o + r] = d.detach().to(device=self.device, dtype=self.dtype)
                bs[:, o : o + r] = (u.detach().to(device=self.device, dtype=torch.float32) * s).to(self.dtype)
                o += r
            if row_perm is not None:
                bs = bs[row_perm].contiguous()
            pack = LoraPack(a, bs)
            R = native.lora_rank(rt)
            if R and self.device.type != "meta":
                ar = torch.zeros(R, k_in, device=self.device, dtype=self.dtype)
                ar[: min(R, rpad)] = a[: min(R, rpad)]
                br = torch.zeros(n_out, R, device=self.device, dtype=self.dtype)
                br[:, : min(R, rpad)] = bs[:, : min(R, rpad)]
                pack.a_kb = native.KBlocked(ar)
                pack.bs_r = br
            return pack

        self.stats["lora_sites"] += 1
        return self.cache.get(key, make)

    def linear_spec(self, node: Any, geglu: bool = False) -> LinSpec:
        if isa(node, "Conv2d") and not isa(node, "LoraAdapter"):
            _expect(node.kernel_size == (1, 1) and node.stride == (1, 1), "only 1x1 convs can act as Linear")
            w = self.cache.get(("conv1x1",) + PackCache.ident(node.weight), lambda: self.cvt(node.weight.detach().reshape(node.out_channels, node.in_channels)))
            return LinSpec(w, self._w(node.bias))
        leaf, loras = self._unwrap_lora(node, "Linear")
        w, b = leaf.weight, leaf.bias
        n_out, k_in = w.shape
        _expect(k_in % self.kblk == 0, f"Linear in_features {k_in} is not a multiple of {self.kblk}")
        perm = None
        if geglu:
            _expect(n_out % 64 == 0, "GEGLU width must be a multiple of 64")
            perm = self.cache.get(("geglu_idx", n_out), lambda: native.geglu_pack_index(n_out // 2, device=self.device))
        if loras and self.lora_mode == "merged":
            downs = [kids(lr)[0].weight for lr in loras]
            ups = [kids(lr)[1].weight for lr in loras]
            scales = tuple(float(kids(lr)[2].scale) for lr in loras)

            def merge() -> Tensor:
                acc = w.detach().to(device=self.device, dtype=torch.float32).clone()
                for d, u, sc in zip(downs, ups, scales):
                    _expect(tuple(d.shape)[1] == k_in and tuple(u.shape)[0] == n_out, "LoRA shape does not match its target")
                    acc = self._mm(u.detach().to(self.device, torch.float32) * sc, d.detach().to(self.device, torch.float32).t(), res=acc)
                acc = acc.to(self.dtype)
                return acc[perm].contiguous() if perm is not None else acc.contiguous()

            wm = self.cache.get(("merged", geglu) + PackCache.ident(w, *downs, *ups) + scales, merge)
            self.stats["lora_sites"] += 1
            bp = None if b is None else (self.cache.get(("geglu_b",) + PackCache.ident(b), lambda: self.cvt(b)[perm].contiguous()) if geglu else self._w(b))
            return LinSpec(wm, bp, None, geglu=geglu)
        if geglu:
            wp = self.cache.get(("geglu_w",) + PackCache.ident(w), lambda: self.cvt(w)[perm].contiguous())
            bp = None if b is None else self.cache.get(("geglu_b",) + PackCache.ident(b), lambda: self.cvt(b)[perm].contiguous())
            return LinSpec(wp, bp, self._lora_pack_linear(loras, n_out, k_in, perm), geglu=True)
        return LinSpec(self._w(w), self._w(b), self._lora_pack_linear(loras, n_out, k_in, None))

    def conv_spec(self, node: Any, asym: bool = False) -> ConvSpec:
        time = None
        if isa(node, "RangeAdapter2d"):
            ch = kids(node)
            _expect(len(ch) == 2 and isa(ch[1], "Chain"), "unexpected RangeAdapter2d layout")
            tc = kids(ch[1])
            _expect(len(tc) == 4 and isa(tc[0], "UseContext") and isa(tc[1], "SiLU") and isa(tc[3], "Reshape"), "unexpected RangeAdapter2d time branch")
            _expect(tc[0].context == "range_adapter", "RangeAdapter2d reads an unexpected context")
            time = (tc[0].key, self.linear_spec(tc[2]))
            node = ch[0]
        leaf, loras = self._unwrap_lora(node, "Conv2d")
        w = leaf.weight
        o, i, kh, kw = w.shape
        _expect(kh == kw and kh in (1, 3), f"conv kernel {kh}x{kw} not supported")
        _expect(leaf.stride[0] == leaf.stride[1] and leaf.stride[0] in (1, 2), "conv stride not supported")
        pad = leaf.padding if isinstance(leaf.padding, tuple) else (leaf.padding, leaf.padding)
        _expect(tuple(pad) == ((0, 0) if asym else (kh // 2, kh // 2)), "only 'same'-style padding k//2 (or Downsample's explicit bottom/right pad) is supported")
        _expect(leaf.groups == 1 and tuple(leaf.dilation) == (1, 1), "grouped / dilated conv not supported")
        _expect((i * self.es) % 128 == 0, f"conv in_channels {i} not 128-byte aligned")
        wp = self.cache.get(("convw",) + PackCache.ident(w), lambda: native.pack_conv_weight(self.cvt(w)))
        lora = None
        def _pad2(c: Any) -> tuple:
            return tuple(c.padding) if isinstance(c.padding, (tuple, list)) else (c.padding, c.padding)

        def mergeable(lr: Any) -> bool:
            d, u = kids(lr)[0], kids(lr)[1]
            return (u.kernel_size == (1, 1) and tuple(u.stride) == (1, 1) and _pad2(u) == (0, 0) and d.kernel_size == (kh, kh)
                    and tuple(d.stride) == tuple(leaf.stride) and _pad2(d) == _pad2(leaf) and tuple(d.dilation) == (1, 1) and d.groups == 1 and u.groups == 1
                    and d.weight.shape[1] == i and u.weight.shape[0] == o and u.weight.shape[1] == d.weight.shape[0])

        if loras and self.lora_mode == "merged" and all(mergeable(lr) for lr in loras):
            dws = [kids(lr)[0].weight for lr in loras]
            uws = [kids(lr)[1].weight for lr in loras]
            scs = tuple(float(kids(lr)[2].scale) for lr in loras)

            def merge_conv() -> Tensor:
                acc = w.detach().to(device=self.device, dtype=torch.float32).clone()
                for d, u, sc in zip(dws, uws, scs):
                    d32 = d.detach().to(self.device, torch.float32)
                    acc = self._mm(u.detach().to(self.device, torch.float32)[:, :, 0, 0] * sc, d32.reshape(d32.shape[0], -1).t(), res=acc.reshape(o, -1)).reshape(acc.shape)
                return native.pack_conv_weight(acc.to(self.dtype))

            wp = self.cache.get(("merged_conv",) + PackCache.ident(w, *dws, *uws) + scs, merge_conv)
            self.stats["lora_sites"] += 1
            loras = []
        if loras:
# ... 34 lines not shown

    def _mm(self, x: Tensor, w: Tensor, res: Optional[Tensor] = None) -> Tensor:
        if self.device.type == "cuda":
            return native.matmul_f32(x.contiguous(), w.contiguous(), None if res is None else res.contiguous())
        y = x @ w.t()
        return y if res is None else y + res

    def lora_sync(self, groups: int, M: int, R: int) -> tuple:
        if self._lsync is None:
            self._lsync = native.LoraSync(self.device)
        if id(self._target) not in self._bumped:
            self._target.insert(0, self._lsync.bump_op())
            self._bumped.add(id(self._target))
        return self.pool.get(native.lora_scratch_rows(groups, M, R, self.dtype), R), self._lsync.flags(groups, M), self._lsync

    def handover_pending(self) -> list:
        out = []
        for st in (self._lsync, self._sk):
            bad = st.pending() if st is not None else None
            if bad is not None:
                out.append(bad)
        return out

    def handover_raise(self) -> None:
        for st in (self._lsync, self._sk):
            if st is not None:
                st.check()

    def colstats_for(self, M: int, N: int, HW: int) -> Any:
        if not self.gn_stats or HW % 32 or N % 16 or self.device.type == "meta" or self._target is self.prologue:
            return None
        cs = torch.empty(native.colstats_shape(M, N), device=self.device, dtype=torch.float32)
        self._cs_buf.append(cs)
        return cs

    def lora_down(self, x: Tensor, lora: LoraPack) -> Tensor:
        t = self.pool.get(x.shape[0], lora.a_cat.shape[0])
        native.gemm([(x, lora.a_cat)], t)
        return t

    def kblocked(self, w: Tensor) -> Any:
        row_bytes = w.shape[1] * w.element_size()
        if self.kblock_policy == 0 or (self.kblock_policy == 1 and row_bytes < 5120) or w.device.type == "meta" or not w.is_contiguous():
            return w
        return self.cache.get(("kblocked",) + PackCache.ident(w), lambda: native.KBlocked(w))

    def linear(self, x: Any, spec: LinSpec, *, res: Optional[Tensor] = None, out: Optional[Tensor] = None,
               rows: Optional[int] = None, lora_t: Optional[Tensor] = None, gelu: bool = False, out_kblocked: bool = False,
               ln: Optional[tuple] = None, stats_out: Optional[Tensor] = None, colstats: Any = None) -> Tensor:
        M = x.shape[0]
        n_cols = spec.N // 2 if spec.geglu else spec.N
        if out is None:
            out = self.pool.get(M, n_cols)
        cso = colstats
        if ln is not None:
            stats, node = ln
            wl, ls, lc = self.ln_fold(spec, node)
            lo = sy = None
            if spec.lora is not None:
                al, als, alc = self.ln_fold_lora(spec.lora, node)
                lo = ([(0, al)], spec.lora.bs_r, als, alc)
                sy = self.lora_sync(1, M, spec.lora.R)
            native.gemm([(x, self.kblocked(wl))], out, res=res, geglu=spec.geglu, gelu=gelu, out_kblocked=out_kblocked, ln=(stats, ls, lc, float(node.eps)),
                        stats_out=stats_out, lora=lo, lora_sync=sy, colstats_out=cso)
            if sy is not None:
                self.pool.put(sy[0])
            return out
        if spec.lora is not None and spec.lora.a_kb is not None and self.lora_inlaunch:
            sy = self.lora_sync(1, M, spec.lora.R)
            native.gemm([(x, self.kblocked(spec.w))], out, bias=spec.b, res=res, geglu=spec.geglu, gelu=gelu, out_kblocked=out_kblocked, stats_out=stats_out,
                        lora=([(0, spec.lora.a_kb)], spec.lora.bs_r), lora_sync=sy, colstats_out=cso)
            self.pool.put(sy[0])
            return out
        segs = [(x, self.kblocked(spec.w))]
        t = None
        if spec.lora is not None:
            t = lora_t if lora_t is not None else self.lora_down(x, spec.lora)
            segs.append((t, spec.lora.bs_cat))
        native.gemm(segs, out, bias=spec.b, res=res, geglu=spec.geglu, gelu=gelu, out_kblocked=out_kblocked, stats_out=stats_out, colstats_out=cso)
        if t is not None and lora_t is None:
            self.pool.put(t)
        return out

    def ln_fold(self, spec: LinSpec, node: Any) -> tuple[Tensor, Tensor, Tensor]:
        _expect(isa(node, "LayerNorm") and tuple(node.normalized_shape) == (spec.K,) and node.weight is not None, "LayerNorm shape mismatch")
        key = ("ln_fold",) + PackCache.ident(spec.w, spec.b, node.weight, node.bias)

        def make() -> tuple[Tensor, Tensor, Tensor]:
            w32 = spec.w.detach().to(self.device, torch.float32)
            g32 = node.weight.detach().to(self.device, torch.float32)
            wl = (w32 * g32.unsqueeze(0)).to(self.dtype).contiguous()
            ls = wl.to(torch.float32).sum(dim=1).contiguous()
            lc = torch.zeros(w32.shape[0], device=self.device, dtype=torch.float32)
            if node.bias is not None:
                lc = self._mm(w32, node.bias.detach().to(self.device, torch.float32).unsqueeze(0)).reshape(-1)
            if spec.b is not None:
                lc = lc + spec.b.detach().to(self.device, torch.float32)
            return wl, ls, lc.contiguous()

        return self.cache.get(key, make)

    def ln_fusable(self, stats: Optional[Tensor], *specs: LinSpec) -> bool:
        ok_lora = lambda sp: sp.lora is None or (sp.lora.a_kb is not None and self.lora_inlaunch)
        return (stats is not None and self.ln_fuse and self.device.type != "meta" and all(ok_lora(sp) and sp.N % 64 == 0 and sp.K % 64 == 0 for sp in specs))

    def ln_fold_lora(self, lora: LoraPack, node: Any) -> tuple[Any, Tensor, Tensor]:
        a = lora.a_kb.dense()
        key = ("ln_fold_lora",) + PackCache.ident(lora.a_cat, node.weight, node.bias)

        def make() -> tuple[Any, Tensor, Tensor]:
            a32 = a.detach().to(self.device, torch.float32)
            g32 = node.weight.detach().to(self.device, torch.float32)
            al = (a32 * g32.unsqueeze(0)).to(self.dtype).contiguous()
            ls = al.to(torch.float32).sum(dim=1).contiguous()
            lc = self._mm(a32, node.bias.detach().to(self.device, torch.float32).unsqueeze(0)).reshape(-1).contiguous() if node.bias is not None else torch.zeros_like(ls)
            return native.KBlocked(al), ls, lc

        return self.cache.get(key, make)

    def row_stats(self, M: int, C: int) -> Optional[Tensor]:
        if not self.ln_fuse or C % 64 or self.device.type == "meta":
            return None
        store = self.__dict__.setdefault("_row_stats", {})
        if (M, C) not in store:
            store[(M, C)] = torch.empty(C // 32, M, 2, device=self.device, dtype=torch.float32)
        return store[(M, C)]

    def linear_T(self, x: Tensor, spec: LinSpec, out_t: Tensor) -> Tensor:
        _expect(spec.b is None, "transposed projection with bias is not supported")
        if spec.lora is not None and spec.lora.a_kb is not None and self.lora_inlaunch and out_t.stride(1) == 1:
            sy = self.lora_sync(1, x.shape[0], spec.lora.R)
            native.gemm([(x, self.kblocked(spec.w))], None, out_t=out_t, nt_begin=0, lora=([(0, spec.lora.a_kb)], spec.lora.bs_r), lora_sync=sy)
            self.pool.put(sy[0])
            return out_t
        segs = [(self.kblocked(spec.w), x)]
        t = None
        if spec.lora is not None:
            t = self.lora_down(x, spec.lora)
            segs.append((spec.lora.bs_cat, t))
        native.gemm(segs, out_t, weight_operand="x")
        self.pool.put(t)
        return out_t

    def conv(self, a: Act, spec: ConvSpec, *, rowbias: Optional[Tensor] = None, res: Optional[Tensor] = None, ups: int = 1,
             shortcut: Optional[tuple[Act, ConvSpec]] = None, bias: Optional[Tensor] = "spec") -> Act:
        H, W = a.H * ups, a.W * ups
        OH, OW = (H + spec.stride - 1) // spec.stride, (W + spec.stride - 1) // spec.stride
        out = self.pool.get(a.B * OH * OW, spec.cout)
        segs = [(a.image(), self.kblocked(spec.w), spec.ksize, spec.stride, ups, int(spec.asym))]
        t = None
        lo = sy = None
        if spec.lora is not None and spec.lora.a_kb is not None and self.lora_inlaunch:
            lo = ([(0, spec.lora.a_kb)], spec.lora.bs_r)
        elif spec.lora is not None:
            kd, ku, st = spec.lora.conv
            t = self.pool.get(a.B * OH * OW, spec.lora.a_cat.shape[0])
            native.conv_gemm([(a.image(), spec.lora.a_cat, kd, st, ups, int(spec.asym))], t, a.B, OH, OW)
            segs.append((Act(t, a.B, OH, OW).image(), spec.lora.bs_cat, ku, 1, 1))
        b = spec.b if isinstance(bias, str) else bias
        if shortcut is not None:
            sa, sspec = shortcut
            _expect(sspec.lora is None and sspec.ksize == 1 and sspec.stride == 1, "unsupported shortcut convolution")
            if isinstance(sa, CatAct):
                c1 = sa.a.C
                w1, w2 = self.cache.get(("sc_split", c1) + PackCache.ident(sspec.w), lambda: (sspec.w[:, :c1].contiguous(), sspec.w[:, c1:].contiguous()))
                segs.append((sa.a.image(), w1, 1, 1, 1))
                segs.append((sa.b.image(), w2, 1, 1, 1))
            else:
                segs.append((sa.image(), sspec.w, 1, 1, 1))
        _expect(len(segs) <= native.MAX_SEG, "too many K segments for one conv launch")
        M_out = a.B * OH * OW
        tiles128 = ((M_out + 127) // 128) * ((spec.cout + 127) // 128)
        total_kb = sum(sg[1].shape[1] for sg in segs) * self.es // 128
        tile, ksplit, ws = 0, 1, None
        if tiles128 <= 192 and total_kb >= 96:
            tile, ksplit = 1, 3
            ws = self.splitk_workspace(ksplit * M_out * spec.cout)
        if lo is not None:
            sy = self.lora_sync(1, M_out, spec.lora.R)
        cs = self.colstats_for(M_out, spec.cout, OH * OW)
# ... 44 lines not shown
```

### refiners_amd/engine/lowering_blocks.py

```python
from __future__ import annotations

import os

import math
from dataclasses import dataclass, field
from typing import Any, Callable, Optional

import torch
import torch.nn.functional as F
from torch import Tensor, nn

from .. import native

from .lowering import Lowering
from .packing import Act, CatAct, ConvSpec, LinSpec, LoraPack, PackCache, Pool, Unsupported, _expect, cname, isa, kids, launches


class BlockLowering(Lowering):
    def _split_attention(self, att: Any, allow_causal: bool = False) -> tuple[list[Any], Any, Any, Optional[Any]]:
        if isa(att, "CrossAttentionAdapter"):
            att = kids(att)[0]
        _expect(isa(att, "Attention"), f"expected an Attention chain, got {cname(att)}")
        ch = [c for c in kids(att) if not isa(c, "SelfAttentionMap")]
        if isa(att, "SelfAttention"):
            _expect(len(ch) == 4 and isa(ch[0], "Parallel") and all(isa(c, "Identity") for c in kids(ch[0])), "unexpected SelfAttention layout")
            ch = ch[1:]
        _expect(len(ch) == 3 and isa(ch[0], "Distribute") and len(kids(ch[0])) == 3, "unexpected Attention layout")
        sd = ch[1]
        ip = None
        if isa(sd, "Sum"):
            sc = kids(sd)
            _expect(len(sc) == 2 and isa(sc[0], "ScaledDotProductAttention") and isa(sc[1], "ImageCrossAttention"), "unexpected Sum around SDPA")
            ip, sd = sc[1], sc[0]
        _expect(isa(sd, "ScaledDotProductAttention") and (allow_causal or not sd.is_causal), "causal or unknown SDPA node")
        _expect(sd.num_heads == att.num_heads, "head count mismatch")
        return kids(ch[0]), sd, ch[2], ip

    def sdpa(self, q: Tensor, B: int, heads: int, streams: list[tuple[Tensor, Tensor, int, float]], v_plain: Optional[list[Tensor]] = None) -> Tensor:
        M, C = q.shape
        Lq = M // B
        out = self.pool.get(M, C)
        d = C // heads
        kind = self.head_kernel(d)
        if kind is not None:
            q3 = q.as_strided((B, Lq, C), (Lq * q.stride(0), q.stride(0), 1))
            st = []
            for k, vt, Lk, osc in streams:
                lkp = k.shape[0] // B
                kv = k.as_strided((B, lkp, C), (lkp * k.stride(0), k.stride(0), 1))
                lv = vt.shape[1] // B
                st.append((kv, vt.as_strided((C, B, lv), (vt.stride(0), lv, 1)), Lk, osc))
            if kind == "flash64":
                native.attention(q3, out.view(B, Lq, C), heads, st)
                return out
            for i, (kv, vt3, Lk, osc) in enumerate(st):
                dst = out if i == 0 else self.pool.get(M, C)
                native.attention_general(q3, kv, vt3, dst.view(B, Lq, C), heads, Lk, out_scale=osc)
                if i > 0:
                    native.axpby(out, 1.0, dst, 1.0, out)
                    self.pool.put(dst)
            return out
        assert v_plain is not None
        kblk = 128 // self.es
        if d % kblk == 0 and all(Lk % kblk == 0 and k.shape[0] == B * Lk for (k, _v, Lk, _o) in streams) and len(streams) == 1 and streams[0][3] == 1.0 and self.device.type != "meta":
            (k, _unused, Lk, osc), v = streams[0], v_plain[0]
            vt = self.pool.get(B * C, Lk)
            native.nhwc_to_nchw(v.view(B, Lk, C), vt.view(B, C, Lk, 1), C)
            scores = self.__dict__.setdefault("_wide_scores", {})
            if (Lq, Lk) not in scores:
                scores[(Lq, Lk)] = (torch.empty(Lq, Lk, device=self.device, dtype=torch.float32), torch.empty(Lq, Lk, device=self.device, dtype=self.dtype))
            sc, pr = scores[(Lq, Lk)]
            for b in range(B):
                for hh in range(heads):
                    qb = q[b * Lq : (b + 1) * Lq, hh * d : (hh + 1) * d]
                    kb = k[b * Lk : (b + 1) * Lk, hh * d : (hh + 1) * d]
                    native.gemm([(qb, kb)], sc, out_f32=self.dtype != torch.float32)
                    native.softmax_rows(sc, pr, Lk, d ** -0.5)
                    vtb = vt.view(B, C, Lk)[b, hh * d : (hh + 1) * d]
                    ob = out[b * Lq : (b + 1) * Lq, hh * d : (hh + 1) * d]
                    native.gemm([(pr, vtb)], ob)
            self.pool.put(vt)
            return out

        def run() -> None:
            acc = None
            for (k, _vt, Lk, osc), v in zip(streams, v_plain):
                lkp = k.shape[0] // B
                qh = q.view(B, Lq, heads, d).transpose(1, 2)
                kh = k.view(B, lkp, heads, d)[:, :Lk].transpose(1, 2)
                vh = v.view(B, lkp, heads, d)[:, :Lk].transpose(1, 2)
                y = F.scaled_dot_product_attention(qh, kh, vh).transpose(1, 2).reshape(M, C)
                acc = y * osc if acc is None else acc + y * osc
            out.copy_(acc)

        self.python(run, f"torch_sdpa_d{d}")
        self.stats["fallback_nodes"].append(f"SDPA(head_dim={d})")
        return out

    def head_kernel(self, d: int) -> Optional[str]:
        if d == 64:
            return "flash64"
        es = 4 if self.dtype == torch.float32 else 2
        if d <= 160 and (d * es) % 16 == 0 and d % 4 == 0:
            return "general"
        return None

    @staticmethod
    def _pad_keys(n: int) -> int:
        return (n + 63) // 64 * 64

    def project_kv(self, src: Tensor, B: int, k_node: Any, v_node: Any, heads: int) -> tuple[Tensor, Tensor, Optional[Tensor]]:
        ks, vs = self.linear_spec(k_node), self.linear_spec(v_node)
        _expect(ks.b is None and vs.b is None, "key / value projections with bias are not supported")
        C = ks.N
        k = self.pool.get(src.shape[0], C)
        self.pool.pin(k)
        self.linear(src, ks, out=k)
        if self.head_kernel(C // heads) is not None:
            vt = self.pool.get(C, src.shape[0])
            self.pool.pin(vt)
            self.linear_T(src, vs, vt)
            return k, vt, None
        v = self.pool.get(src.shape[0], C)
        self.pool.pin(v)
        self.linear(src, vs, out=v)
        return k, v, v

    def _project_vt(self, h: Tensor, vs: LinSpec, B: int, L: int, C: int) -> Tensor:
        if L % 64 == 0:
            vt = self.pool.get(C, B * L)
            self.linear_T(h, vs, vt)
            return vt
        lp = (L + 63) // 64 * 64
        vt = torch.zeros(C, B * lp, device=self.device, dtype=self.dtype)
        self.__dict__.setdefault("_keep", []).append(vt)
        for b in range(B):
            self.linear_T(h[b * L : (b + 1) * L], vs, vt[:, b * lp : b * lp + L])
        return vt

    def self_attention(self, x: Tensor, B: int, ln: Any, att: Any, stats: Optional[Tensor] = None, stats_out: Optional[Tensor] = None) -> Tensor:
        (qn, kn, vn), sd, on, ip = self._split_attention(att)
        _expect(ip is None, "image cross-attention on a self-attention")
        heads = sd.num_heads
        qs, ks, vs = self.linear_spec(qn), self.linear_spec(kn), self.linear_spec(vn)
        _expect(qs.b is None and ks.b is None and vs.b is None, "q/k/v bias not supported")
        M, C = x.shape
        native_path = self.head_kernel(C // heads) is not None
        L = M // B
        fold = self.ln_fusable(stats, qs, ks, vs)
        lnarg = (stats, ln) if fold else None
        h = x if fold else self.layernorm(x, ln)
        no_lora = qs.lora is None and ks.lora is None and vs.lora is None
        all_inlaunch = self.lora_inlaunch and all(sp.lora is not None and sp.lora.a_kb is not None for sp in (qs, ks, vs)) and len({sp.lora.R for sp in (qs, ks, vs)}) == 1
        qk = q = k = vt = None
        if (no_lora or all_inlaunch) and native_path and self.qkv_merge and L % 64 == 0 and C % 128 == 0 and self.device.type != "meta":
            wqkv = LinSpec(self.cache.get(("qkv",) + PackCache.ident(qs.w, ks.w, vs.w), lambda: torch.cat([qs.w, ks.w, vs.w], 0).contiguous()), None)
            qk = self.pool.get(M, 2 * C)
            vt = self.pool.get(C, M)
            if fold:
                wl, ls, lc = self.ln_fold(wqkv, ln)
                lo = sy = None
                if not no_lora:
                    packs = [self.ln_fold_lora(sp.lora, ln) for sp in (qs, ks, vs)]
                    bs = self.cache.get(("qkv_bs",) + PackCache.ident(qs.lora.bs_r, ks.lora.bs_r, vs.lora.bs_r), lambda: torch.cat([qs.lora.bs_r, ks.lora.bs_r, vs.lora.bs_r], 0).contiguous())
                    sy = self.lora_sync(3, M, qs.lora.R)
                    lsc = self.cache.get(("qkv_lsc",) + PackCache.ident(*[t for pk in packs for t in pk[1:]]), lambda: (torch.cat([pk[1] for pk in packs]).contiguous(), torch.cat([pk[2] for pk in packs]).contiguous()))
                    lo = ([(0, packs[0][0]), (C, packs[1][0]), (2 * C, packs[2][0])], bs, lsc[0], lsc[1])
                native.gemm([(h, self.kblocked(wl))], qk, out_t=vt, nt_begin=2 * C, ln=(stats, ls, lc, float(ln.eps)), lora=lo, lora_sync=sy)
                if sy is not None:
                    self.pool.put(sy[0])
            elif no_lora:
                native.gemm([(h, self.kblocked(wqkv.w))], qk, out_t=vt, nt_begin=2 * C)
            else:
                bs = self.cache.get(("qkv_bs",) + PackCache.ident(qs.lora.bs_r, ks.lora.bs_r, vs.lora.bs_r), lambda: torch.cat([qs.lora.bs_r, ks.lora.bs_r, vs.lora.bs_r], 0).contiguous())
                sy = self.lora_sync(3, M, qs.lora.R)
                native.gemm([(h, self.kblocked(wqkv.w))], qk, out_t=vt, nt_begin=2 * C, lora=([(0, qs.lora.a_kb), (C, ks.lora.a_kb), (2 * C, vs.lora.a_kb)], bs), lora_sync=sy)
                self.pool.put(sy[0])
            q, k = qk[:, :C], qk[:, C:]
        else:
            if fold and (not (native_path and L % 64 == 0) or not no_lora):
                h, lnarg, fold = self.layernorm(x, ln), None, False
            if qs.lora is None and ks.lora is None:
                wqk = LinSpec(self.cache.get(("qk",) + PackCache.ident(qs.w, ks.w), lambda: torch.cat([qs.w, ks.w], 0).contiguous()), None)
                qk = self.linear(h, wqk, ln=lnarg)
                q, k = qk[:, :C], qk[:, C:]
            else:
                q = self.linear(h, qs)
                k = self.linear(h, ks)
            if native_path:
                if fold:
                    vt = self.pool.get(C, M)
                    wl, ls, lc = self.ln_fold(vs, ln)
                    native.gemm([(h, self.kblocked(wl))], None, out_t=vt, nt_begin=0, ln=(stats, ls, lc, float(ln.eps)))
                else:
                    vt = self._project_vt(h, vs, B, L, C)
        tap = next((c for c in kids(att) if isa(c, "SelfAttentionMap")), None)
        if tap is not None and getattr(self, "sag_capture", True):
            self.sag_attention_mass(q, k, B, heads, L, C)
        if native_path:
            o = self.sdpa(q, B, heads, [(k, vt, L, 1.0)])
            if L % 64 == 0:
                self.pool.put(vt)
        else:
            v = self.linear(h, vs)
            o = self.sdpa(q, B, heads, [(k, v, M // B, 1.0)], v_plain=[v])
            self.pool.put(v)
        if h is not x:
            self.pool.put(h)
        if qk is not None:
            self.pool.put(qk)
        else:
            self.pool.put(q)
            self.pool.put(k)
        self.linear(o, self.linear_spec(on), res=x, out=x, stats_out=stats_out)
        self.pool.put(o)
        return x

    def sag_attention_mass(self, q: Tensor, k: Tensor, B: int, heads: int, L: int, C: int) -> None:
        d = C // heads
        kblk = 128 // self.es
        _expect(d % kblk == 0 and B % 2 == 0, "self-attention guidance tap: head width / batch not supported")
        n = B // 2
        mass = torch.zeros(n, L, device=self.device, dtype=torch.float32)
        sc = torch.empty(L, L, device=self.device, dtype=torch.float32)
        pr = torch.empty(L, L, device=self.device, dtype=self.dtype)
        self.__dict__.setdefault("_keep", []).extend([mass, sc, pr])
        if self.device.type != "meta":
            for b in range(n):
                for h in range(heads):
                    qb, kb = q[b * L : (b + 1) * L, h * d : (h + 1) * d], k[b * L : (b + 1) * L, h * d : (h + 1) * d]
                    native.gemm([(qb, kb)], sc, out_f32=self.dtype != torch.float32)
                    native.softmax_rows(sc, pr, L, d ** -0.5)
                    native.colsum_rows(pr, mass[b], accumulate=h > 0, scale=1.0 / heads)
        self.sag = {"mass": mass, "tokens": L}

    def cross_attention(self, x: Tensor, B: int, ln: Any, par: Any, att: Any, ctx: "UNetContext", stats: Optional[Tensor] = None,
                        stats_out: Optional[Tensor] = None) -> Tensor:
        pc = kids(par)
        _expect(len(pc) == 3 and isa(pc[0], "Identity") and all(isa(c, "UseContext") for c in pc[1:]), "unexpected cross-attention Parallel")
        _expect(pc[1].context == pc[2].context and pc[1].key == pc[2].key, "key and value read different contexts")
        (qn, kn, vn), sd, on, ip = self._split_attention(att)
        heads = sd.num_heads
        src, Lk = ctx.tokens(pc[1].context, pc[1].key)
        with self.in_prologue():
            k, v_or_vt, v_plain = self.project_kv(src, B, kn, vn, heads)
        streams = [(k, v_or_vt, Lk, 1.0)]
        plains = [v_plain]
        if ip is not None:
            ic = kids(ip)
            _expect(len(ic) == 3 and isa(ic[0], "Distribute") and isa(ic[1], "ScaledDotProductAttention") and isa(ic[2], "Multiply"), "unexpected ImageCrossAttention layout")
            dc = kids(ic[0])
            _expect(len(dc) == 3 and isa(dc[0], "Identity"), "unexpected ImageCrossAttention Distribute")
            kc, vc = kids(dc[1]), kids(dc[2])
            _expect(len(kc) == 2 and len(vc) == 2 and isa(kc[0], "UseContext") and isa(vc[0], "UseContext"), "unexpected image K/V branch")
            _expect(ic[2].bias == 0.0 and ic[1].num_heads == heads, "unexpected ImageCrossAttention parameters")
            isrc, ilk = ctx.tokens(kc[0].context, kc[0].key)
            with self.in_prologue():
                k2, v2, vp2 = self.project_kv(isrc, B, kc[1], vc[1], heads)
            streams.append((k2, v2, ilk, float(ic[2].scale)))
            plains.append(vp2)
            self.stats["ip_sites"] += 1
        qspec = self.linear_spec(qn)
        M, C = x.shape[0], qspec.N
        if self.ln_fusable(stats, qspec):
            q = self.linear(x, qspec, ln=(stats, ln))
        else:
            h = self.layernorm(x, ln)
            q = self.linear(h, qspec)
            self.pool.put(h)
        o = self.sdpa(q, B, heads, streams, v_plain=plains if plains[0] is not None else None)
        self.pool.put(q)
        self.linear(o, self.linear_spec(on), res=x, out=x, stats_out=stats_out)
        self.pool.put(o)
        return x

    def feed_forward(self, x: Tensor, ln: Any, w1: Any, glu: Any, w2: Any, stats: Optional[Tensor] = None, stats_out: Optional[Tensor] = None) -> Tensor:
        _expect(isa(glu, "GLU") and isa(glu.activation, "GeLU") and glu.activation.approximation.value == "none", "only GLU(GeLU(exact)) is fused")
        s1, s2 = self.linear_spec(w1, geglu=True), self.linear_spec(w2)
        inl = lambda sp: sp.lora is None or (sp.lora.a_kb is not None and self.lora_inlaunch)
        blocked = self.kblock_policy > 0 and inl(s1) and inl(s2) and s1.N % 256 == 0 and self.device.type != "meta"
        if self.ln_fusable(stats, s1):
            ff = self.linear(x, s1, out_kblocked=blocked, ln=(stats, ln))
        else:
# ... 108 lines not shown
```

### refiners_amd/native.py

```python
from __future__ import annotations

import ctypes as C
import os
import weakref
from pathlib import Path
from typing import Any, Optional, Sequence

import torch
from torch import Tensor

MI355X_F32 = 0
MI355X_BF16 = 1
MAX_SEG = 3

_ERR = {0: "OK", -1: "EDTYPE", -2: "ESHAPE", -3: "ELAUNCH", -4: "EARG"}

LIB_PATH = Path(__file__).resolve().parent / "csrc" / "libmi355x_refiners.so"


class NativeError(RuntimeError):
    """Raised when the native library is unavailable or a native call returns a negative status."""


class GemmSeg(C.Structure):
# ... 66 lines not shown
        ("dtype", C.c_int32),
        ("M", C.c_int32),
        ("N", C.c_int32),
        ("nseg", C.c_int32),
        ("conv", C.c_int32),
        ("B", C.c_int32),
        ("OH", C.c_int32),
        ("OW", C.c_int32),
        ("seg", GemmSeg * MAX_SEG),
        ("out", C.c_void_p),
        ("ldo", C.c_int64),
        ("bias", C.c_void_p),
        ("rowbias", C.c_void_p),
        ("ld_rowbias", C.c_int64),
        ("rows_per_group", C.c_int32),
        ("geglu", C.c_int32),
        ("res", C.c_void_p),
        ("ldres", C.c_int64),
        ("zeros", C.c_void_p),
        ("tile", C.c_int32),
        ("ksplit", C.c_int32),
        ("ws", C.c_void_p),
        ("ws_bytes", C.c_int64),
        ("prefetch", C.c_void_p * MAX_PREFETCH),
        ("prefetch_bytes", C.c_int64 * MAX_PREFETCH),
        ("prefetch_blocks", C.c_int32),
        ("out_kblocked", C.c_int32),
        ("stages", C.c_int32),
        ("nt_begin", C.c_int32),
        ("out_t", C.c_void_p),
        ("ldt", C.c_int64),
        ("ln_stats", C.c_void_p),
        ("ln_parts", C.c_int32),
        ("ln_eps", C.c_float),
        ("ln_s", C.c_void_p),
        ("ln_c", C.c_void_p),
        ("stats_out", C.c_void_p),
        ("out_f32", C.c_int32),
        ("lora_a", C.c_void_p * 3),
        ("lora_nb", C.c_int32 * 3),
        ("lora_groups", C.c_int32),
        ("lora_r", C.c_int32),
        ("lora_b", C.c_void_p),
        ("lora_ls", C.c_void_p),
        ("lora_lc", C.c_void_p),
        ("lora_t", C.c_void_p),
        ("lora_flags", C.c_void_p),
        ("lora_epoch", C.c_void_p),
        ("colstats_out", C.c_void_p),
        ("sk_ws", C.c_void_p),
        ("sk_flags", C.c_void_p),
        ("sk_slots", C.c_int32),
    ]


class KvStream(C.Structure):
    _fields_ = [
        ("k", C.c_void_p),
        ("ldk", C.c_int64),
        ("k_batch_stride", C.c_int64),
        ("vt", C.c_void_p),
        ("ldvt", C.c_int64),
        ("vt_batch_stride", C.c_int64),
        ("Lk", C.c_int32),
        ("out_scale", C.c_float),
    ]


class AttnArgs(C.Structure):
    _fields_ = [
        ("dtype", C.c_int32),
        ("B", C.c_int32),
        ("H", C.c_int32),
        ("D", C.c_int32),
        ("Lq", C.c_int32),
        ("nstream", C.c_int32),
        ("q", C.c_void_p),
        ("ldq", C.c_int64),
        ("q_batch_stride", C.c_int64),
        ("out", C.c_void_p),
        ("ldo", C.c_int64),
        ("o_batch_stride", C.c_int64),
        ("scale", C.c_float),
        ("kv", KvStream * 2),
    ]


class AttnGeneralArgs(C.Structure):
    _fields_ = [
        ("dtype", C.c_int32),
        ("B", C.c_int32),
        ("H", C.c_int32),
        ("Lq", C.c_int32),
        ("Lk", C.c_int32),
        ("Dqk", C.c_int32),
        ("Dv", C.c_int32),
        ("causal", C.c_int32),
        ("q", C.c_void_p),
        ("ldq", C.c_int64),
        ("q_batch_stride", C.c_int64),
        ("k", C.c_void_p),
        ("ldk", C.c_int64),
        ("k_batch_stride", C.c_int64),
        ("vt", C.c_void_p),
        ("ldvt", C.c_int64),
        ("vt_batch_stride", C.c_int64),
        ("out", C.c_void_p),
        ("ldo", C.c_int64),
        ("o_batch_stride", C.c_int64),
        ("scale", C.c_float),
        ("out_scale", C.c_float),
    ]


class LayerNormArgs(C.Structure):
    _fields_ = [
        ("dtype", C.c_int32),
        ("M", C.c_int32),
        ("C", C.c_int32),
        ("x", C.c_void_p),
        ("ldx", C.c_int64),
        ("gamma", C.c_void_p),
        ("beta", C.c_void_p),
        ("eps", C.c_float),
        ("out", C.c_void_p),
        ("ldo", C.c_int64),
    ]


class GroupNormArgs(C.Structure):
    _fields_ = [
        ("dtype", C.c_int32),
        ("B", C.c_int32),
        ("HW", C.c_int32),
        ("C", C.c_int32),
        ("G", C.c_int32),
        ("x", C.c_void_p),
        ("ldx", C.c_int64),
        ("gamma", C.c_void_p),
        ("beta", C.c_void_p),
        ("eps", C.c_float),
        ("silu", C.c_int32),
        ("out", C.c_void_p),
        ("ldo", C.c_int64),
        ("ws", C.c_void_p),
        ("colstats", C.c_void_p),
        ("x2", C.c_void_p),
        ("ldx2", C.c_int64),
        ("C1", C.c_int32),
        ("colstats2", C.c_void_p),
    ]



class SamAttnArgs(C.Structure):
    _fields_ = [
        ("dtype", C.c_int32), ("B", C.c_int32), ("H", C.c_int32), ("D", C.c_int32), ("Lq", C.c_int32), ("Lk", C.c_int32),
        ("q", C.c_void_p), ("ldq", C.c_int64), ("q_batch_stride", C.c_int64),
        ("k", C.c_void_p), ("ldk", C.c_int64), ("k_batch_stride", C.c_int64),
        ("v", C.c_void_p), ("ldv", C.c_int64), ("v_batch_stride", C.c_int64),
        ("out", C.c_void_p), ("ldo", C.c_int64), ("o_batch_stride", C.c_int64),
        ("scale", C.c_float), ("ws", C.c_void_p), ("ws_floats", C.c_int64),
    ]


class SamMaskHeadArgs(C.Structure):
# ... 25 lines not shown
    "mi355x_nchw_to_nhwc",
    "mi355x_nhwc_to_nchw",
    "mi355x_im2col3x3_nchw",
    "mi355x_concat2",
    "mi355x_axpby",
    "mi355x_silu",
    "mi355x_softmax_rows",
    "mi355x_colsum_rows",
    "mi355x_sag_degrade",
    "mi355x_cfg_ddim_step",
    "mi355x_cfg_linear_step",
    "mi355x_sinusoidal",
    "mi355x_patchify_nchw",
    "mi355x_gather_rows",
    "mi355x_pointwise_nchw",
    "mi355x_relpos_pack",
    "mi355x_sam_attention",
    "mi355x_convt2x2_ln_gelu",
    "mi355x_sam_mask_head",
    "mi355x_sam_postprocess_masks",
]

_lib: Optional[C.CDLL] = None
_lib_path: Optional[str] = None


def load(path: Optional[Path] = None) -> C.CDLL:
    global _lib, _lib_path
    if _lib is not None:
        return _lib
    p = Path(path) if path else Path(os.environ.get("REFINERS_AMD_LIB") or LIB_PATH)
    if not p.exists():
        raise NativeError(
            f"{p} is missing: build it with `python -m refiners_amd.build_native` (or __graft_entry__.build()). "
            "There is no fallback path for the MI355X kernels."
        )
    try:
        lib = C.CDLL(str(p))
    except OSError as e:
        raise NativeError(f"cannot load {p}: {e}") from e
    lib.mi355x_abi_version.restype = C.c_int
    if os.environ.get("REFINERS_AMD_FORCE_TILE"):
        lib.mi355x_set_option(b"tile", int(os.environ["REFINERS_AMD_FORCE_TILE"]))
    lib.mi355x_device_info.argtypes = [C.c_char_p, C.c_int32]
    lib.mi355x_gemm.argtypes = [C.POINTER(GemmArgs), C.c_void_p]
    lib.mi355x_epoch_bump.argtypes = [C.c_void_p, C.c_void_p]
    lib.mi355x_attention.argtypes = [C.POINTER(AttnArgs), C.c_void_p]
    lib.mi355x_attention_general.argtypes = [C.POINTER(AttnGeneralArgs), C.c_void_p]
    lib.mi355x_layernorm.argtypes = [C.POINTER(LayerNormArgs), C.c_void_p]
    lib.mi355x_groupnorm.argtypes = [C.POINTER(GroupNormArgs), C.c_void_p]
    lib.mi355x_groupnorm_ws_floats.argtypes = [C.c_int32, C.c_int32, C.c_int32]
    lib.mi355x_groupnorm_ws_floats.restype = C.c_int64
    lib.mi355x_nchw_to_nhwc.argtypes = [C.c_int32, C.c_void_p, C.c_void_p, C.c_int32, C.c_int32, C.c_int32, C.c_int64, C.c_void_p]
    lib.mi355x_nhwc_to_nchw.argtypes = [C.c_int32, C.c_void_p, C.c_void_p, C.c_int32, C.c_int32, C.c_int32, C.c_int64, C.c_void_p]
    lib.mi355x_im2col3x3_nchw.argtypes = [C.c_int32, C.c_void_p, C.c_void_p, C.c_int32, C.c_int32, C.c_int32, C.c_int32, C.c_int64, C.c_void_p]
    lib.mi355x_concat2.argtypes = [C.c_int32, C.c_void_p, C.c_int64, C.c_int32, C.c_void_p, C.c_int64, C.c_int32, C.c_void_p, C.c_int64, C.c_int64, C.c_void_p]
    lib.mi355x_axpby.argtypes = [C.c_int32, C.c_void_p, C.c_float, C.c_void_p, C.c_float, C.c_void_p, C.c_int64, C.c_void_p]
    lib.mi355x_silu.argtypes = [C.c_int32, C.c_void_p, C.c_void_p, C.c_int64, C.c_void_p]
    lib.mi355x_colsum_rows.argtypes = [C.c_int32, C.c_void_p, C.c_int64, C.c_int32, C.c_int32, C.c_void_p, C.c_int32, C.c_float, C.c_void_p]
    lib.mi355x_sag_degrade.argtypes = [C.c_int32, C.c_void_p, C.c_void_p, C.c_void_p, C.c_int32, C.c_int32, C.c_void_p, C.c_void_p, C.c_int32, C.c_void_p, C.c_int32, C.c_int32,
                                       C.c_int32, C.c_int32, C.c_void_p]
    lib.mi355x_softmax_rows.argtypes = [C.c_int32, C.c_void_p, C.c_int64, C.c_void_p, C.c_int64, C.c_int64, C.c_int32, C.c_int32, C.c_float, C.c_void_p]
    lib.mi355x_cfg_ddim_step.argtypes = [C.c_int32, C.c_void_p, C.c_void_p, C.c_void_p, C.c_int64, C.c_void_p]
    lib.mi355x_cfg_linear_step.argtypes = [C.c_int32, C.c_void_p, C.c_void_p, C.c_void_p, C.c_void_p, C.c_void_p, C.c_int64, C.c_void_p]
    lib.mi355x_sinusoidal.argtypes = [C.c_int32, C.c_void_p, C.c_int64, C.c_int32, C.c_int32, C.c_void_p, C.c_int64, C.c_int32, C.c_void_p]
    lib.mi355x_patchify_nchw.argtypes = [C.c_int32, C.c_void_p, C.c_void_p, C.c_int32, C.c_int32, C.c_int32, C.c_int32, C.c_int32, C.c_int64, C.c_void_p]
    lib.mi355x_gather_rows.argtypes = [C.c_int32, C.c_void_p, C.c_int64, C.c_void_p, C.c_void_p, C.c_int64, C.c_int64, C.c_int32, C.c_void_p]
    lib.mi355x_pointwise_nchw.argtypes = [C.c_int32, C.c_void_p, C.c_void_p, C.c_void_p, C.c_void_p, C.c_int32, C.c_int32, C.c_int32, C.c_int64, C.c_void_p]
    lib.mi355x_relpos_pack.argtypes = [C.c_int32, C.c_void_p, C.c_int64, C.c_void_p, C.c_int64, C.c_int64, C.c_int32, C.c_int32, C.c_int32, C.c_int32, C.c_int32, C.c_int32, C.c_void_p]
    lib.mi355x_sam_attention.argtypes = [C.POINTER(SamAttnArgs), C.c_void_p]
    lib.mi355x_convt2x2_ln_gelu.argtypes = [C.c_int32, C.c_void_p, C.c_int64, C.c_int64, C.c_int32, C.c_int32, C.c_void_p, C.c_void_p, C.c_float, C.c_void_p,
                                            C.c_int64, C.c_int32, C.c_int32, C.c_void_p]
    lib.mi355x_sam_mask_head.argtypes = [C.POINTER(SamMaskHeadArgs), C.c_void_p]
    lib.mi355x_sam_postprocess_masks.argtypes = [C.POINTER(SamPostprocessArgs), C.c_void_p]
    lib.mi355x_set_option.argtypes = [C.c_char_p, C.c_int]
    lib.mi355x_attention_set_glds.argtypes = [C.c_int]
    lib.mi355x_attention_general_set_fast.argtypes = [C.c_int]
    lib.mi355x_attention_set_pipeline.argtypes = [C.c_int, C.c_int]
    if lib.mi355x_abi_version() != 7:
        raise NativeError("libmi355x_refiners.so ABI version mismatch")
    _lib = lib
    _lib_path = str(p)
    attention_pipeline_from_env()
    return lib


def attention_pipeline_from_env() -> None:
    import os

    d, x, o, k, sp, sh = (os.environ.get("REFINERS_AMD_ATTN_PIPE", "").replace("/", ",").split(",") + ["", "", "", "", "", ""])[:6]
    _lib.mi355x_attention_set_pipeline(int(d or 1) | (int(o or 13) << 4) | (int(k or 0) << 16) | (int(sp or 3) << 19) | (int(sh or 0) << 23), int(x or 1))


def available() -> bool:
    try:
        load()
        return True
    except NativeError:
        return False


def switch_library(path: Optional[Path]) -> C.CDLL:
    global _lib
    _lib = None
    return load(path)


def loaded_library_path() -> Optional[str]:
    return _lib_path if _lib is not None else None


def check(status: int, what: str) -> None:
    if status != 0:
        raise NativeError(f"{what} failed with MI355X_{_ERR.get(status, status)}")


def dtype_code(dt: torch.dtype) -> int:
    if dt == torch.float32:
        return MI355X_F32
    if dt == torch.bfloat16:
        return MI355X_BF16
    raise NativeError(f"unsupported dtype {dt} (the MI355X path computes in float32 or bfloat16)")


def stream_ptr() -> int:
    return torch.cuda.current_stream().cuda_stream


def device_info() -> str:
    buf = C.create_string_buffer(256)
    check(load().mi355x_device_info(buf, 256), "mi355x_device_info")
    return buf.value.decode()



_recorder: Optional[list] = None


class recording:

    def __init__(self, ops: list) -> None:
        self.ops = ops

    def __enter__(self) -> list:
        global _recorder
        self._saved = _recorder
        _recorder = self.ops
        return self.ops

    def __exit__(self, *exc: object) -> None:
        global _recorder
        _recorder = self._saved


class not_recording:

    def __enter__(self) -> None:
        global _recorder
        self._saved = _recorder
        _recorder = None

    def __exit__(self, *exc: object) -> None:
        global _recorder
        _recorder = self._saved


def matmul_f32(x: Tensor, w: Tensor, res: Optional[Tensor] = None) -> Tensor:
# ... 379 lines not shown
            self.ws = torch.empty(self.SLOTS * 65536, dtype=torch.float32, device=self.device)
            self.flags = torch.zeros(self.SLOTS + 1, dtype=torch.int32, device=self.device)
        return self.ws, self.flags

    def pending(self) -> Optional[Tensor]:
        return None if self.flags is None else self.flags[-1] != 0

    def check(self) -> None:
        bad = self.pending()
        if bad is not None and bool(bad.item()):
            self.flags.zero_()
            raise NativeError("mi355x_gemm (stream-K): a workgroup's partial tile never arrived (MI355X_ELAUNCH)")


_streamk_current: Optional[StreamK] = None
_streamk_eager: dict[tuple[int, int], StreamK] = {}


def set_streamk(sk: Optional[StreamK]) -> Optional[StreamK]:
    global _streamk_current
    old, _streamk_current = _streamk_current, sk
    return old


def attach_streamk(a: GemmArgs, sk: StreamK) -> None:
    w, f = sk.tensors()
    a.sk_ws, a.sk_flags, a.sk_slots = w.data_ptr(), f.data_ptr(), sk.SLOTS
    a._sk_keep = sk


def _fill_split(a: GemmArgs, tile: int, ksplit: int, ws: Optional[Tensor], stages: int = 0, table_may_replace_split: bool = False, operand: Optional[Tensor] = None) -> None:
    if tile == 0 and ksplit <= 1:
        from .engine import tuning

        tile, stages = tuning.lookup(gemm_signature(a), stages)
    elif ksplit > 1 and table_may_replace_split:
        from .engine import tuning

        t8, _ = tuning.lookup(gemm_signature(a), 0)
        if t8 in (7, 8, 9, 10, 12):
            tile = t8
    a.tile, a.ksplit, a.stages = tile, ksplit, stages
    if tile == 8 or os.environ.get("REFINERS_AMD_FORCE_TILE") == "8":
        sk = _streamk_current
        if sk is None:
            dev = operand.device if operand is not None and operand.device.type == "cuda" else torch.device("cuda", torch.cuda.current_device())
            if dev.index is None:
                dev = torch.device("cuda", torch.cuda.current_device())
            key = (dev.index, torch.cuda.current_stream(dev).cuda_stream)
            sk = _streamk_eager.get(key)
            if sk is None:
                sk = _streamk_eager[key] = StreamK(dev)
        attach_streamk(a, sk)
    if ksplit > 1:
        assert ws is not None and ws.is_contiguous(), "split-K needs a scratch tensor of ksplit * M * N float32"
        a.ws, a.ws_bytes = ws.data_ptr(), ws.numel() * ws.element_size()
    else:
        a.ws, a.ws_bytes = None, 0


def _fill_epilogue(a: GemmArgs, out: Tensor, bias, rowbias, rows_per_group, res, geglu) -> None:
    assert out.dim() == 2 and out.stride(1) == 1
    a.out, a.ldo = out.data_ptr(), out.stride(0)
    a.bias = bias.data_ptr() if bias is not None else None
    if rowbias is not None:
        assert rowbias.dim() == 2 and rowbias.stride(1) == 1
        a.rowbias, a.ld_rowbias, a.rows_per_group = rowbias.data_ptr(), rowbias.stride(0), rows_per_group
    else:
        a.rowbias, a.ld_rowbias, a.rows_per_group = None, 0, 1
    if res is not None:
        assert res.dim() == 2 and res.stride(1) == 1
        a.res, a.ldres = res.data_ptr(), res.stride(0)
    else:
        a.res, a.ldres = None, 0
    a.geglu = int(geglu)


def attention(
    q: Tensor,
    out: Tensor,
    num_heads: int,
    streams: Sequence[tuple[Tensor, Tensor, int, float]],
    scale: Optional[float] = None,
) -> Tensor:
    a = AttnArgs()
    B, Lq, HD = q.shape
    D = HD // num_heads
    a.dtype = dtype_code(q.dtype)
    a.B, a.H, a.D, a.Lq, a.nstream = B, num_heads, D, Lq, len(streams)
    assert q.stride(2) == 1 and out.stride(2) == 1
    a.q, a.ldq, a.q_batch_stride = q.data_ptr(), q.stride(1), q.stride(0)
    a.out, a.ldo, a.o_batch_stride = out.data_ptr(), out.stride(1), out.stride(0)
    a.scale = scale if scale is not None else D ** -0.5
    for s, (k, vt, Lk, osc) in enumerate(streams):
        assert k.dim() == 3 and vt.dim() == 3 and k.stride(2) == 1 and vt.stride(2) == 1
        kv = a.kv[s]
        kv.k, kv.ldk, kv.k_batch_stride = k.data_ptr(), k.stride(1), k.stride(0)
        kv.vt, kv.ldvt, kv.vt_batch_stride = vt.data_ptr(), vt.stride(0), vt.stride(1)
        kv.Lk, kv.out_scale = Lk, osc
    _launch("mi355x_attention", (C.byref(a),), "mi355x_attention")
    return out


def attention_general(
    q: Tensor,
    k: Tensor,
    vt: Tensor,
    out: Tensor,
    num_heads: int,
    Lk: int,
    scale: Optional[float] = None,
    causal: bool = False,
    out_scale: float = 1.0,
) -> Tensor:
    a = AttnGeneralArgs()
    B, Lq, HD = q.shape
    assert HD % num_heads == 0 and vt.shape[0] % num_heads == 0 and out.shape[2] == vt.shape[0]
    assert q.stride(2) == 1 and k.stride(2) == 1 and vt.stride(2) == 1 and out.stride(2) == 1
    a.dtype = dtype_code(q.dtype)
    a.B, a.H, a.Lq, a.Lk = B, num_heads, Lq, Lk
    a.Dqk, a.Dv, a.causal = HD // num_heads, vt.shape[0] // num_heads, int(causal)
    a.q, a.ldq, a.q_batch_stride = q.data_ptr(), q.stride(1), q.stride(0)
    a.k, a.ldk, a.k_batch_stride = k.data_ptr(), k.stride(1), k.stride(0)
    a.vt, a.ldvt, a.vt_batch_stride = vt.data_ptr(), vt.stride(0), vt.stride(1)
    a.out, a.ldo, a.o_batch_stride = out.data_ptr(), out.stride(1), out.stride(0)
    a.scale = scale if scale is not None else a.Dqk ** -0.5
    a.out_scale = out_scale
    _launch("mi355x_attention_general", (C.byref(a),), "mi355x_attention_general")
    return out


def layernorm(x: Tensor, gamma: Tensor, beta: Tensor, eps: float, out: Tensor) -> Tensor:
    a = LayerNormArgs()
    assert x.dim() == 2 and out.dim() == 2 and x.stride(1) == 1 and out.stride(1) == 1
    a.dtype = dtype_code(x.dtype)
    a.M, a.C = x.shape
    a.x, a.ldx, a.gamma, a.beta, a.eps = x.data_ptr(), x.stride(0), gamma.data_ptr(), beta.data_ptr(), eps
    a.out, a.ldo = out.data_ptr(), out.stride(0)
    _launch("mi355x_layernorm", (C.byref(a),), "mi355x_layernorm")
    return out


_gn_ws: "weakref.WeakValueDictionary[tuple[int, int, int], Tensor]" = weakref.WeakValueDictionary()


def groupnorm_nhwc(x: Tensor, gamma: Tensor, beta: Tensor, groups: int, eps: float, silu: bool, out: Tensor, colstats: Optional[Tensor] = None,
                   x2: Optional[Tensor] = None, colstats2: Optional[Tensor] = None) -> Tensor:
    a = GroupNormArgs()
    B, HW, C1 = x.shape
    Cc = C1 + (x2.shape[2] if x2 is not None else 0)
    assert x.stride(2) == 1 and out.stride(2) == 1 and x.stride(0) == HW * x.stride(1) and out.stride(0) == HW * out.stride(1) and out.shape[2] == Cc
    if x2 is not None:
        assert x2.shape[:2] == x.shape[:2] and x2.stride(2) == 1 and x2.stride(0) == HW * x2.stride(1) and x2.dtype == x.dtype and (colstats is None) == (colstats2 is None)
        a.x2, a.ldx2, a.C1 = x2.data_ptr(), x2.stride(1), C1
    need = load().mi355x_groupnorm_ws_floats(B, HW, Cc)
    if x.device.type == "cuda":
        dev = x.device.index if x.device.index is not None else torch.cuda.current_device()
        key = (dev, torch.cuda.current_stream().cuda_stream, id(_recorder) if _recorder is not None else 0)
    else:
        key = (-1, 0, 0)
    ws = _gn_ws.get(key)
    if ws is None or ws.numel() < need:
        ws = torch.empty(max(need, 1 << 20), dtype=torch.float32, device=x.device)
        _gn_ws[key] = ws
    a.dtype = dtype_code(x.dtype)
    a.B, a.HW, a.C, a.G = B, HW, Cc, groups
    a.x, a.ldx, a.gamma, a.beta, a.eps, a.silu = x.data_ptr(), x.stride(1), gamma.data_ptr(), beta.data_ptr(), eps, int(silu)
    a.out, a.ldo, a.ws = out.data_ptr(), out.stride(1), ws.data_ptr()
    if colstats is not None:
        assert HW % 32 == 0 and colstats.dtype == torch.float32 and colstats.is_contiguous() and colstats.numel() >= B * HW // 32 * C1 * 2
        a.colstats = colstats.data_ptr()
        if colstats2 is not None:
            assert colstats2.dtype == torch.float32 and colstats2.is_contiguous() and colstats2.numel() >= B * HW // 32 * (Cc - C1) * 2
            a.colstats2 = colstats2.data_ptr()
    _launch("mi355x_groupnorm", (C.byref(a),), "mi355x_groupnorm", keep=(ws, colstats, x2, colstats2))
    return out
# ... 196 lines not shown
```

Measured before the change: 0.8687 images/s.

## Fold attention softmax scale into K projection weights and add shared LoRA producers

Self-attention K projection weights, biases and LoRA up-weights are pre-multiplied by the softmax scale times log2(e), so the attention kernel can use c=1 and a new FOLD=2 variant that skips in-kernel scaling. It also adds an optional shared LoRA producer mode (off unless REFINERS_AMD_LORA_SHARED is set) where one block computes all stacked LoRA groups for 32 or 64 rows. LayerNorm stat merging in the producer switches to fixed-contraction FMA. Folding the scale into bf16 K weights changes rounding slightly.

Result: no change. 0.8716 images/s (median of 6 runs) (+0.3%).

```diff
diff --git a/include/mi355x_refiners.h b/include/mi355x_refiners.h
--- a/include/mi355x_refiners.h
+++ b/include/mi355x_refiners.h
@@ -116,6 +116,7 @@
     int64_t ldo;
     int64_t o_batch_stride;
     float scale;
+    int32_t k_prescaled;
     mi355x_kv_stream kv[2];
 } mi355x_attn_args;
 
diff --git a/refiners_amd/csrc/attention.hip b/refiners_amd/csrc/attention.hip
--- a/refiners_amd/csrc/attention.hip
+++ b/refiners_amd/csrc/attention.hip
@@ -24,6 +24,7 @@
     KvP kv[2];
     int qtiles;
     int xcd;
+    int kpre;
 };
 
 MI_DEV void xswap16(float& a, float& b) { asm("s_nop 1\n\tv_permlane16_swap_b32 %0, %1" : "+v"(a), "+v"(b)); }
@@ -494,7 +495,7 @@
     __builtin_amdgcn_raw_ptr_buffer_load_lds(rs, (lptr_t)lds_wave_base, 16, (int)voff, (int)soff, 0, 0);
 }
 
-template <int NJQ, int SCHED, int ABL = 0, bool DMA = false, bool FOLD = false>
+template <int NJQ, int SCHED, int ABL = 0, bool DMA = false, int FOLD = 0>
 __global__ __launch_bounds__(256) __attribute__((amdgpu_waves_per_eu(2))) void attn_pipe_kernel(const AttnP p) {
     using T = bf16_t;
     constexpr int NW = 4, D = 64, BKV = 64, BQW = 16 * NJQ, ES = 2, ROWB = D * ES, CPR = ROWB / 16, NTHR = NW * 64, TILEB = 64 * ROWB;
@@ -519,7 +520,7 @@
 #pragma unroll
         for (int s = 0; s < NS; ++s) {
             qf[jq][s] = *reinterpret_cast<const frag_t*>(qp + (4 * s + g) * 16);
-            if constexpr (FOLD) {
+            if constexpr (FOLD == 1) {
                 bf16x8 qv = __builtin_bit_cast(bf16x8, qf[jq][s]);
 #pragma unroll
                 for (int e = 0; e < 8; ++e) qv[e] = (bf16_t)((float)qv[e] * p.c);
@@ -1288,7 +1289,7 @@
 
 int g_attn_pipe_fold = 0;
 
-template <int NJQ, int SCHED, int ABL = 0, bool DMA = false, bool FOLD = false>
+template <int NJQ, int SCHED, int ABL = 0, bool DMA = false, int FOLD = 0>
 int launch_attn_pipe(const AttnP& p0, hipStream_t stream) {
     constexpr int LDS = 4 * 64 * 64 * 2;
     auto kfn = attn_pipe_kernel<NJQ, SCHED, ABL, DMA, FOLD>;
@@ -1381,7 +1382,8 @@
             if (g_attn_pipe == 2) return q16 ? launch_attn_pipe<1, 0>(p, stream) : launch_attn_pipe<2, 0>(p, stream);
             if (g_attn_pipe == 3) {
                 const bool dma_ok = (int64_t)p.kv[0].Lk * p.kv[0].ldkb < 0x7fffffff && 64 * p.kv[0].ldvtb < 0x7fffffff;
-                if (dma_ok && g_attn_pipe_fold) return q16 ? launch_attn_pipe<1, 1, 0, true, true>(p, stream) : launch_attn_pipe<2, 1, 0, true, true>(p, stream);
+                if (dma_ok && p.kpre) return q16 ? launch_attn_pipe<1, 1, 0, true, 2>(p, stream) : launch_attn_pipe<2, 1, 0, true, 2>(p, stream);
+                if (dma_ok && g_attn_pipe_fold) return q16 ? launch_attn_pipe<1, 1, 0, true, 1>(p, stream) : launch_attn_pipe<2, 1, 0, true, 1>(p, stream);
                 if (dma_ok) return q16 ? launch_attn_pipe<1, 1, 0, true>(p, stream) : launch_attn_pipe<2, 1, 0, true>(p, stream);
             }
             return q16 ? launch_attn_pipe<1, 1>(p, stream) : launch_attn_pipe<2, 1>(p, stream);
@@ -1490,7 +1492,8 @@
     p.out = static_cast<char*>(a->out);
     p.ldob = a->ldo * es;
     p.obsb = a->o_batch_stride * es;
-    p.c = a->scale * 1.44269504088896340736f;
+    p.kpre = a->k_prescaled != 0;
+    p.c = p.kpre ? 1.0f : a->scale * 1.44269504088896340736f;
     p.thr = p.c > 0.f ? 8.0f / p.c : 0.f;
     for (int s = 0; s < a->nstream; ++s) {
         const mi355x_kv_stream& k = a->kv[s];
diff --git a/refiners_amd/csrc/gemm.hip b/refiners_amd/csrc/gemm.hip
--- a/refiners_amd/csrc/gemm.hip
+++ b/refiners_amd/csrc/gemm.hip
@@ -10,6 +10,8 @@
 int g_tile = 0;
 int g_stages = 0;
 int g_lora_dbg = 0;
+int g_lora_shared = 0;
+int g_stat_lora_shared = 0;
 int g_sk_g = 0;
 int g_g8_persist = 1;
 
@@ -47,6 +49,11 @@
         else g_pf_mode = value;
         return MI355X_OK;
     }
+    if (name[0] == 'l' && name[1] == 's') {
+        if (value != 0 && value != 32 && value != 64) return MI355X_EARG;
+        g_lora_shared = value;
+        return MI355X_OK;
+    }
     if (name[0] == 'l') {
         g_lora_dbg = value;
         return MI355X_OK;
@@ -62,6 +69,7 @@
 extern "C" int mi355x_get_stat(const char* name);
 extern "C" int mi355x_get_stat(const char* name) {
     if (!name) return MI355X_EARG;
+    if (name[0] == 'l' && name[1] == 's') return g_stat_lora_shared;
     if (name[0] == 'g' && name[1] == '8') return name[2] == 'l' ? g_stat_g8_lora : g_stat_g8;
     if (name[0] == 'g' && name[1] == '9') return g_stat_g9;
     if (name[0] == 'g' && name[1] == '1' && name[2] == '1') return g_stat_g11;
diff --git a/refiners_amd/csrc/gemm_epilogue.cuh b/refiners_amd/csrc/gemm_epilogue.cuh
--- a/refiners_amd/csrc/gemm_epilogue.cuh
+++ b/refiners_amd/csrc/gemm_epilogue.cuh
@@ -431,6 +431,8 @@
 extern int g_tile;
 extern int g_stages;
 extern int g_lora_dbg;
+extern int g_lora_shared;
+extern int g_stat_lora_shared;
 
 
 inline void plan_grid(GemmP& q, int BM, int BN, bool conv, int kg) {
diff --git a/refiners_amd/csrc/gemm_kernel.cuh b/refiners_amd/csrc/gemm_kernel.cuh
--- a/refiners_amd/csrc/gemm_kernel.cuh
+++ b/refiners_amd/csrc/gemm_kernel.cuh
@@ -19,6 +19,14 @@
 template <typename T, int BM, int BN, bool LORA> constexpr int gemm_min_waves() {
     if (!LORA || sizeof(T) != 2) return 1;
     return BM * BN == 128 * 128 ? 2 : BM * BN == 64 * 64 ? MI355X_LORA64_WAVES : BM == 128 ? 3 : 2;
+}
+
+constexpr int lora_shared_stage(int pm, int stacked) { return (pm + stacked) * 128; }
+
+template <typename T, int RI, int PM, int RING>
+__device__ __forceinline__ void lora_shared_producer(const GemmP& p, int q) {
+    constexpr int PS = RING / lora_shared_stage(PM, 32 * RI);
+    if constexpr (PS >= 2) lora_producer<T, false, RI, (PS < 8 ? PS : 8), PM, true>(p, q);
 }
 
 template <typename T, int BM, int BN, int WM, int WN, bool CONV, int NSTAGE, int KG = 1, bool LORA = false>
@@ -82,6 +90,25 @@
         if (!ttile && bid < p.lp_blocks) {
             if ((p.lora_dbg & 1) || bid >= (p.M + LORA_PM - 1) / LORA_PM * p.lora_groups) return;
             constexpr int RING = KG * NSTAGE * (BM + BN) * 128;
+            if constexpr (!CONV) {
+                if (p.lora_sp) {
+                    if ((p.lora_dbg & 1) || bid >= (p.M + p.lora_sp - 1) / p.lora_sp) return;
+                    const __attribute__((address_space(4))) GemmP* pe = (const __attribute__((address_space(4))) GemmP*)__builtin_amdgcn_kernarg_segment_ptr();
+                    asm volatile("" : "+s"(pe));
+                    const GemmP& pk = *(const GemmP*)pe;
+                    const int ri = p.lora_groups * p.lora_r / 32;
+                    if (p.lora_sp == 64) {
+                        if (ri == 2) lora_shared_producer<T, 2, 64, RING>(pk, bid);
+                        else if (ri == 3) lora_shared_producer<T, 3, 64, RING>(pk, bid);
+                        else lora_shared_producer<T, 4, 64, RING>(pk, bid);
+                    } else {
+                        if (ri == 2) lora_shared_producer<T, 2, 32, RING>(pk, bid);
+                        else if (ri == 3) lora_shared_producer<T, 3, 32, RING>(pk, bid);
+                        else lora_shared_producer<T, 4, 32, RING>(pk, bid);
+                    }
+                    return;
+                }
+            }
             constexpr int PB1 = (LORA_PM + 32) * 128, PB2 = (LORA_PM + 64) * 128, PB4 = (LORA_PM + 128) * 128;
             constexpr int P1 = RING / PB1 < 8 ? RING / PB1 : 8, P2 = RING / PB2 < 8 ? RING / PB2 : 8, P4 = RING / PB4;
             if (p.lora_r == 32) lora_producer<T, CONV, 1, P1>(p, bid);
@@ -570,11 +597,17 @@
     plan_grid(q, BM, BN, CONV, KG);
     q.lora_dbg = g_lora_dbg;
     q.lora_tt = 0;
+    q.lora_sp = 0;
     if constexpr (LORA && !CONV && KG == 1) {
+        constexpr int RING = KG * NSTAGE * (BM + BN) * 128;
+        const int stacked = q.lora_groups * q.lora_r;
+        int sp = (g_lora_dbg & (64 | 128 | 256)) ? 0 : g_lora_shared;
+        if (sp && q.lora_groups > 1 && q.nseg == 1 && q.ksplit <= 1 && stacked <= LORA_RMAX && stacked % 32 == 0 && RING / lora_shared_stage(sp, stacked) >= 2) q.lora_sp = sp;
         const int mode = (g_lora_dbg & 64) ? 0 : (g_lora_dbg & 128) ? 2 : MI355X_LORA_TT;
-        if (q.lora_groups * q.lora_r <= BN && q.ksplit <= 1 && q.nseg == 1 && (mode == 2 || (mode == 1 && q.lora_groups > 1))) q.lora_tt = 1;
-    }
-    q.lp_blocks = !LORA ? 0 : q.lora_tt ? (q.tiles_m + 7) / 8 * 8 : ((q.M + LORA_PM - 1) / LORA_PM * q.lora_groups + 7) / 8 * 8;
+        if (!q.lora_sp && stacked <= BN && q.ksplit <= 1 && q.nseg == 1 && (mode == 2 || (mode == 1 && q.lora_groups > 1))) q.lora_tt = 1;
+    }
+    if (q.lora_sp) ++g_stat_lora_shared;
+    q.lp_blocks = !LORA ? 0 : q.lora_tt ? (q.tiles_m + 7) / 8 * 8 : q.lora_sp ? ((q.M + q.lora_sp - 1) / q.lora_sp + 7) / 8 * 8 : ((q.M + LORA_PM - 1) / LORA_PM * q.lora_groups + 7) / 8 * 8;
     const int grid = q.pf_blocks + q.lp_blocks + q.grid0 * (q.ksplit > 1 ? q.ksplit : 1);
     hipLaunchKernelGGL(kfn, dim3(grid), dim3(WM * WN * 64 * KG), q.ln_stats ? LDS : LDS - BM * 8, stream, q);
     if (q.ksplit > 1) {
diff --git a/refiners_amd/csrc/gemm_lora_producer.cuh b/refiners_amd/csrc/gemm_lora_producer.cuh
--- a/refiners_amd/csrc/gemm_lora_producer.cuh
+++ b/refiners_amd/csrc/gemm_lora_producer.cuh
@@ -7,15 +7,30 @@
 constexpr int LORA_PM = 32;
 constexpr int LORA_RMAX = 128;
 
-template <typename T, bool CONV, int RI, int PST>
+MI_DEV void stat_merge_fixed(float& n, float& mean, float& m2, float nb, float mb, float m2b) {
+#pragma clang fp contract(off)
+    const float nt = n + nb;
+    if (nt > 0.f) {
+        const float d = mb - mean, f = nb / nt;
+        mean = __builtin_fmaf(d, f, mean);
+        const float dd = d * d, ddn = dd * n;
+        m2 = m2 + __builtin_fmaf(ddn, f, m2b);
+        n = nt;
+    }
+}
+
+template <typename T, bool CONV, int RI, int PST, int PM = LORA_PM, bool SHARED = false>
 __device__ __forceinline__ void lora_producer(const GemmP& p, int q, int tid_in = -1, char* lds = nullptr) {
     extern __shared__ __attribute__((aligned(16))) char smem_all[];
     char* const smem = lds ? lds : smem_all;
-    constexpr int NTHR = 256, PXB = LORA_PM * 128, PSTAGE = PXB + 32 * RI * 128, PD = PST - 1, PL = 1 + RI;
+    constexpr int NTHR = 256, XL = PM / 32, PXB = PM * 128, PSTAGE = PXB + 32 * RI * 128, PD = PST - 1, PL = XL + RI;
+    constexpr int NRB = PM / 16, NJ = 2 * RI * NRB / 4;
     static_assert(PST >= 2 && PST <= 8, "LoRA producer: 2..8 stages");
+    static_assert(PM == 32 || (SHARED && PM == 64), "LoRA producer: 32 rows, shared producers 32 or 64");
+    static_assert(!(SHARED && CONV), "shared LoRA producers: plain GEMMs only");
     const int tid = tid_in >= 0 ? tid_in : (int)threadIdx.x, lane = tid & 63, wid = __builtin_amdgcn_readfirstlane(tid >> 6), g = lane >> 4, c16 = lane & 15;
-    const int npb = (p.M + LORA_PM - 1) / LORA_PM;
-    const int pgi = q / npb, tm = q - pgi * npb, m0 = tm * LORA_PM;
+    const int npb = (p.M + PM - 1) / PM;
+    const int pgi = SHARED ? 0 : q / npb, tm = q - pgi * npb, m0 = tm * PM;
     const int tag = *p.lora_epoch;
     if (p.lora_dbg & 32) __builtin_amdgcn_s_setprio(3);
     const SegP& sp = p.seg[0];
@@ -49,11 +64,22 @@
     };
     if constexpr (CONV) set_tap();
     else xbase = sp.x + (sp.xkb ? (int64_t)xm * 128 : (int64_t)xm * sp.ldxb) + xcoff;
+    const char* xbase2 = nullptr;
+    if constexpr (XL == 2) {
+        const int row2 = row + 32, xm2 = m0 + row2 < p.M ? m0 + row2 : p.M - 1;
+        xbase2 = sp.x + (sp.xkb ? (int64_t)xm2 * 128 : (int64_t)xm2 * sp.ldxb) + ((pch ^ swz<128>(row2)) << 4);
+    }
     const char* pw[RI];
 #pragma unroll
     for (int j = 0; j < RI; ++j) {
         const int qq = j * NTHR + tid, r = qq >> 3, c = qq & 7;
-        pw[j] = p.lora_a[pgi] + (int64_t)r * 128 + ((c ^ swz<128>(r)) << 4);
+        if constexpr (SHARED) {
+            const int gi = r / p.lora_r;
+            const char* ag = gi == 0 ? p.lora_a[0] : gi == 1 ? p.lora_a[1] : p.lora_a[2];
+            pw[j] = ag + (int64_t)(r - gi * p.lora_r) * 128 + ((c ^ swz<128>(r)) << 4);
+        } else {
+            pw[j] = p.lora_a[pgi] + (int64_t)r * 128 + ((c ^ swz<128>(r)) << 4);
+        }
     }
     int kb = 0;
     auto issue_p = [&](int buf) __attribute__((always_inline)) {
@@ -62,6 +88,7 @@
         if constexpr (CONV) src = xbase ? xbase + (int64_t)cb * 128 : p.zeros + xcoff;
         else src = xbase + xoff;
         glds16(src, st + wid * 64 * 16);
+        if constexpr (XL == 2) glds16(xbase2 + xoff, st + (NTHR + wid * 64) * 16);
 #pragma unroll
         for (int j = 0; j < RI; ++j) glds16(pw[j] + woff, st + PXB + (j * NTHR + wid * 64) * 16);
         ++kb;
@@ -76,7 +103,7 @@
             xoff += xstep;
         }
     };
-    const int rb = wid & 1, rg = wid >> 1;
+    const int rb = wid % NRB, rg = wid / NRB;
     const int mrow = 16 * rb + c16, m = m0 + mrow;
     float mean = 0.f, inv = 1.f;
     constexpr int MAXP = 48;
@@ -91,19 +118,20 @@
     for (int s0 = 0; s0 < PD; ++s0)
         if (s0 < nkb) issue_p(s0);
     if (sp2) {
+#pragma clang fp contract(off)
         float m2 = 0.f, cn = 0.f;
 #pragma unroll
         for (int i = 0; i < MAXP; ++i)
-            if (i < p.ln_parts) stat_merge(cn, mean, m2, 32.f, lst[i][0], lst[i][1]);
+            if (i < p.ln_parts) stat_merge_fixed(cn, mean, m2, 32.f, lst[i][0], lst[i][1]);
         for (int part = MAXP; part < p.ln_parts; ++part) {
             const f32x2 s2 = *reinterpret_cast<const f32x2*>(sp2 + part * pstride);
-            stat_merge(cn, mean, m2, 32.f, s2[0], s2[1]);
+            stat_merge_fixed(cn, mean, m2, 32.f, s2[0], s2[1]);
         }
         inv = sqrtf(m2 / cn + p.ln_eps);
     }
-    f32x4 ta[RI];
+    f32x4 ta[NJ];
 #pragma unroll
-    for (int j = 0; j < RI; ++j) ta[j] = f32x4{0.f, 0.f, 0.f, 0.f};
+    for (int j = 0; j < NJ; ++j) ta[j] = f32x4{0.f, 0.f, 0.f, 0.f};
     for (int t = 0; t < nkb; ++t) {
         if (t + PD <= nkb) wait_vm<(PD - 1) * PL>();
         else wait_vm0();
@@ -115,21 +143,22 @@
         for (int kk = 0; kk < 2; ++kk) {
             const frag_t xf = lds_read_frag(st, tile_off<128>(16 * rb + c16, 4 * kk + g));
 #pragma unroll
-            for (int j = 0; j < RI; ++j) {
-                const frag_t af = lds_read_frag(st + PXB, tile_off<128>((rg * RI + j) * 16 + c16, 4 * kk + g));
+            for (int j = 0; j < NJ; ++j) {
+                const frag_t af = lds_read_frag(st + PXB, tile_off<128>((rg * NJ + j) * 16 + c16, 4 * kk + g));
                 mma_step<T>(ta[j], af, xf);
             }
         }
     }
-    char* tg = p.lora_t + pgi * p.lora_gs;
 #pragma unroll
-    for (int j = 0; j < RI; ++j) {
-        const int r0 = (rg * RI + j) * 16 + 4 * g;
+    for (int j = 0; j < NJ; ++j) {
+        const int s0 = (rg * NJ + j) * 16 + 4 * g;
+        const int sgi = SHARED ? s0 / p.lora_r : pgi, r0 = SHARED ? s0 - sgi * p.lora_r : s0;
+        char* tg = p.lora_t + sgi * p.lora_gs;
         f32x4 v = ta[j];
         if (p.ln_stats) {
-            const f32x4 sa = *reinterpret_cast<const f32x4*>(p.lora_ls + pgi * p.lora_r + r0), ca = *reinterpret_cast<const f32x4*>(p.lora_lc + pgi * p.lora_r + r0);
+            const f32x4 sa = *reinterpret_cast<const f32x4*>(p.lora_ls + sgi * p.lora_r + r0), ca = *reinterpret_cast<const f32x4*>(p.lora_lc + sgi * p.lora_r + r0);
 #pragma unroll
-            for (int e = 0; e < 4; ++e) v[e] = (v[e] - mean * sa[e]) + ca[e] * inv;
+            for (int e = 0; e < 4; ++e) v[e] = __builtin_fmaf(ca[e], inv, __builtin_fmaf(-mean, sa[e], v[e]));
         }
         if (m < p.M) {
             char* dst = tg + ((int64_t)m * p.lora_r + r0) * (int)sizeof(T);
@@ -144,7 +173,12 @@
     }
     asm volatile("s_waitcnt vmcnt(0)" ::: "memory");
     __syncthreads();
-    if (tid == 0) __hip_atomic_store(p.lora_flags + pgi * npb + tm, tag, __ATOMIC_RELAXED, __HIP_MEMORY_SCOPE_AGENT);
+    if constexpr (SHARED) {
+        const int nfl = (p.M + 31) / 32, gi = tid / XL, blk = tm * XL + tid % XL;
+        if (tid < p.lora_groups * XL && blk < nfl) __hip_atomic_store(p.lora_flags + gi * nfl + blk, tag, __ATOMIC_RELAXED, __HIP_MEMORY_SCOPE_AGENT);
+    } else {
+        if (tid == 0) __hip_atomic_store(p.lora_flags + pgi * npb + tm, tag, __ATOMIC_RELAXED, __HIP_MEMORY_SCOPE_AGENT);
+    }
 }
 
 }
diff --git a/refiners_amd/csrc/gemm_params.cuh b/refiners_amd/csrc/gemm_params.cuh
--- a/refiners_amd/csrc/gemm_params.cuh
+++ b/refiners_amd/csrc/gemm_params.cuh
@@ -63,6 +63,7 @@
     const int* lora_epoch;
     int lp_blocks;
     int lora_tt;
+    int lora_sp;
     int64_t lora_gs;
     int lora_dbg;
     const char* pf_ptr[MI355X_MAX_PREFETCH];
diff --git a/refiners_amd/engine/lowering.py b/refiners_amd/engine/lowering.py
--- a/refiners_amd/engine/lowering.py
+++ b/refiners_amd/engine/lowering.py
@@ -22,6 +22,7 @@
         self.kblock_policy = int(os.environ.get("REFINERS_AMD_KBLOCK", "2"))
         self.ln_fuse = os.environ.get("REFINERS_AMD_LN_FUSE", "1") != "0"
         self.qkv_merge = os.environ.get("REFINERS_AMD_QKV_MERGE", "1") != "0"
+        self.attn_kfold = os.environ.get("REFINERS_AMD_ATTN_KFOLD", "1") != "0"
         self.lora_inlaunch = os.environ.get("REFINERS_AMD_LORA_INLAUNCH", "1") != "0"
         self.gn_stats = os.environ.get("REFINERS_AMD_GN_STATS", "1") != "0"
         self._cs_buf: list[Tensor] = []
@@ -124,6 +125,22 @@
 
         self.stats["lora_sites"] += 1
         return self.cache.get(key, make)
+
+    def lora_up_scaled(self, node: Any, pack: LoraPack, factor: float) -> Tensor:
+        _, loras = self._unwrap_lora(node, "Linear")
+        ups = [kids(lr)[1].weight for lr in loras]
+        scales = tuple(float(kids(lr)[2].scale) for lr in loras)
+
+        def make() -> Tensor:
+            br = torch.zeros_like(pack.bs_r)
+            o = 0
+            for u, s in zip(ups, scales):
+                r = u.shape[1]
+                br[:, o : o + r] = (u.detach().to(device=self.device, dtype=torch.float32) * s * factor).to(self.dtype)
+                o += r
+            return br
+
+        return self.cache.get(("lora_up_scaled",) + PackCache.ident(*ups) + scales + (float(factor),), make)
 
     def linear_spec(self, node: Any, geglu: bool = False) -> LinSpec:
         if isa(node, "Conv2d") and not isa(node, "LoraAdapter"):
@@ -324,12 +341,15 @@
             self.pool.put(t)
         return out
 
-    def ln_fold(self, spec: LinSpec, node: Any) -> tuple[Tensor, Tensor, Tensor]:
+    def ln_fold(self, spec: LinSpec, node: Any, row_scale: Optional[tuple[int, int, float]] = None) -> tuple[Tensor, Tensor, Tensor]:
         _expect(isa(node, "LayerNorm") and tuple(node.normalized_shape) == (spec.K,) and node.weight is not None, "LayerNorm shape mismatch")
-        key = ("ln_fold",) + PackCache.ident(spec.w, spec.b, node.weight, node.bias)
+        key = ("ln_fold",) + PackCache.ident(spec.w, spec.b, node.weight, node.bias) + (() if row_scale is None else ("row_scale",) + tuple(row_scale))
 
         def make() -> tuple[Tensor, Tensor, Tensor]:
             w32 = spec.w.detach().to(self.device, torch.float32)
+            if row_scale is not None:
+                w32 = w32.clone()
+                w32[row_scale[0] : row_scale[1]] *= row_scale[2]
             g32 = node.weight.detach().to(self.device, torch.float32)
             wl = (w32 * g32.unsqueeze(0)).to(self.dtype).contiguous()
             ls = wl.to(torch.float32).sum(dim=1).contiguous()
@@ -337,7 +357,11 @@
             if node.bias is not None:
                 lc = self._mm(w32, node.bias.detach().to(self.device, torch.float32).unsqueeze(0)).reshape(-1)
             if spec.b is not None:
-                lc = lc + spec.b.detach().to(self.device, torch.float32)
+                b32 = spec.b.detach().to(self.device, torch.float32)
+                if row_scale is not None:
+                    b32 = b32.clone()
+                    b32[row_scale[0] : row_scale[1]] *= row_scale[2]
+                lc = lc + b32
             return wl, ls, lc.contiguous()
 
         return self.cache.get(key, make)
diff --git a/refiners_amd/engine/lowering_blocks.py b/refiners_amd/engine/lowering_blocks.py
--- a/refiners_amd/engine/lowering_blocks.py
+++ b/refiners_amd/engine/lowering_blocks.py
@@ -36,7 +36,8 @@
         _expect(sd.num_heads == att.num_heads, "head count mismatch")
         return kids(ch[0]), sd, ch[2], ip
 
-    def sdpa(self, q: Tensor, B: int, heads: int, streams: list[tuple[Tensor, Tensor, int, float]], v_plain: Optional[list[Tensor]] = None) -> Tensor:
+    def sdpa(self, q: Tensor, B: int, heads: int, streams: list[tuple[Tensor, Tensor, int, float]], v_plain: Optional[list[Tensor]] = None,
+             k_prescaled: bool = False) -> Tensor:
         M, C = q.shape
         Lq = M // B
         out = self.pool.get(M, C)
@@ -51,7 +52,7 @@
                 lv = vt.shape[1] // B
                 st.append((kv, vt.as_strided((C, B, lv), (vt.stride(0), lv, 1)), Lk, osc))
             if kind == "flash64":
-                native.attention(q3, out.view(B, Lq, C), heads, st)
+                native.attention(q3, out.view(B, Lq, C), heads, st, k_prescaled=k_prescaled)
                 return out
             for i, (kv, vt3, Lk, osc) in enumerate(st):
                 dst = out if i == 0 else self.pool.get(M, C)
@@ -153,16 +154,21 @@
         no_lora = qs.lora is None and ks.lora is None and vs.lora is None
         all_inlaunch = self.lora_inlaunch and all(sp.lora is not None and sp.lora.a_kb is not None for sp in (qs, ks, vs)) and len({sp.lora.R for sp in (qs, ks, vs)}) == 1
         qk = q = k = vt = None
+        tap = next((c for c in kids(att) if isa(c, "SelfAttentionMap")), None)
+        sag = tap is not None and getattr(self, "sag_capture", True)
+        kfold = self.attn_kfold and fold and self.dtype == torch.bfloat16 and C // heads == 64 and L > 3 * 64 and not sag
+        kc = (C // heads) ** -0.5 * 1.4426950408889634
         if (no_lora or all_inlaunch) and native_path and self.qkv_merge and L % 64 == 0 and C % 128 == 0 and self.device.type != "meta":
             wqkv = LinSpec(self.cache.get(("qkv",) + PackCache.ident(qs.w, ks.w, vs.w), lambda: torch.cat([qs.w, ks.w, vs.w], 0).contiguous()), None)
             qk = self.pool.get(M, 2 * C)
             vt = self.pool.get(C, M)
             if fold:
-                wl, ls, lc = self.ln_fold(wqkv, ln)
+                wl, ls, lc = self.ln_fold(wqkv, ln, row_scale=(C, 2 * C, kc) if kfold else None)
                 lo = sy = None
                 if not no_lora:
                     packs = [self.ln_fold_lora(sp.lora, ln) for sp in (qs, ks, vs)]
-                    bs = self.cache.get(("qkv_bs",) + PackCache.ident(qs.lora.bs_r, ks.lora.bs_r, vs.lora.bs_r), lambda: torch.cat([qs.lora.bs_r, ks.lora.bs_r, vs.lora.bs_r], 0).contiguous())
+                    kbs = self.lora_up_scaled(kn, ks.lora, kc) if kfold else ks.lora.bs_r
+                    bs = self.cache.get(("qkv_bs",) + PackCache.ident(qs.lora.bs_r, kbs, vs.lora.bs_r), lambda: torch.cat([qs.lora.bs_r, kbs, vs.lora.bs_r], 0).contiguous())
                     sy = self.lora_sync(3, M, qs.lora.R)
                     lsc = self.cache.get(("qkv_lsc",) + PackCache.ident(*[t for pk in packs for t in pk[1:]]), lambda: (torch.cat([pk[1] for pk in packs]).contiguous(), torch.cat([pk[2] for pk in packs]).contiguous()))
                     lo = ([(0, packs[0][0]), (C, packs[1][0]), (2 * C, packs[2][0])], bs, lsc[0], lsc[1])
@@ -178,6 +184,7 @@
                 self.pool.put(sy[0])
             q, k = qk[:, :C], qk[:, C:]
         else:
+            kfold = False
             if fold and (not (native_path and L % 64 == 0) or not no_lora):
                 h, lnarg, fold = self.layernorm(x, ln), None, False
             if qs.lora is None and ks.lora is None:
@@ -194,11 +201,10 @@
                     native.gemm([(h, self.kblocked(wl))], None, out_t=vt, nt_begin=0, ln=(stats, ls, lc, float(ln.eps)))
                 else:
                     vt = self._project_vt(h, vs, B, L, C)
-        tap = next((c for c in kids(att) if isa(c, "SelfAttentionMap")), None)
-        if tap is not None and getattr(self, "sag_capture", True):
+        if sag:
             self.sag_attention_mass(q, k, B, heads, L, C)
         if native_path:
-            o = self.sdpa(q, B, heads, [(k, vt, L, 1.0)])
+            o = self.sdpa(q, B, heads, [(k, vt, L, 1.0)], k_prescaled=kfold)
             if L % 64 == 0:
                 self.pool.put(vt)
         else:
diff --git a/refiners_amd/native.py b/refiners_amd/native.py
--- a/refiners_amd/native.py
+++ b/refiners_amd/native.py
@@ -172,6 +172,7 @@
         ("ldo", C.c_int64),
         ("o_batch_stride", C.c_int64),
         ("scale", C.c_float),
+        ("k_prescaled", C.c_int32),
         ("kv", KvStream * 2),
     ]
 
@@ -363,7 +364,17 @@
     _lib = lib
     _lib_path = str(p)
     attention_pipeline_from_env()
+    lora_shared_from_env()
     return lib
+
+
+def lora_shared_from_env() -> None:
+    import os
+
+    rows = int(os.environ.get("REFINERS_AMD_LORA_SHARED", "") or 0)
+    if rows != getattr(_lib, "_lsrows", 0):
+        check(_lib.mi355x_set_option(b"lsrows", rows), "mi355x_set_option lsrows")
+        _lib._lsrows = rows
 
 
 def attention_pipeline_from_env() -> None:
@@ -909,6 +920,7 @@
     num_heads: int,
     streams: Sequence[tuple[Tensor, Tensor, int, float]],
     scale: Optional[float] = None,
+    k_prescaled: bool = False,
 ) -> Tensor:
     a = AttnArgs()
     B, Lq, HD = q.shape
@@ -919,6 +931,7 @@
     a.q, a.ldq, a.q_batch_stride = q.data_ptr(), q.stride(1), q.stride(0)
     a.out, a.ldo, a.o_batch_stride = out.data_ptr(), out.stride(1), out.stride(0)
     a.scale = scale if scale is not None else D ** -0.5
+    a.k_prescaled = int(k_prescaled)
     for s, (k, vt, Lk, osc) in enumerate(streams):
         assert k.dim() == 3 and vt.dim() == 3 and k.stride(2) == 1 and vt.stride(2) == 1
         kv = a.kv[s]
```
